# VincentGourbin/ltx-video-swift-mlx

Measured on NVIDIA B200. Metric: dit_steps_per_s, higher is better.
Workload: dtype bf16

## Files before the change

ltx-video-swift-mlx_b200/csrc/api.cu:

```cuda
#include <cstring>

#include "ctx.h"

using namespace ltx;

namespace {

thread_local std::string g_create_error;

template <typename Fn>
int guarded(ltx_ctx* c, Fn&& fn) {
  if (!c) return LTX_ERR_INVALID_ARGUMENT;
  try {
    LTX_CUDA(cudaSetDevice(c->device));
    fn();
    return LTX_OK;
  } catch (const LtxError& e) {
    c->last_error = e.what();
    return e.code;
  } catch (const std::exception& e) {
    c->last_error = e.what();
    return LTX_ERR_CUDA;
  }
}
// ... 63 lines not shown
  }
  if (it == c->graphs.end()) {
    if (c->graphs.size() >= 8) {
      auto lru = c->graphs.begin();
      for (auto j = c->graphs.begin(); j != c->graphs.end(); ++j)
        if (j->second.last_use < lru->second.last_use) lru = j;
      graph_destroy(lru->second);
      c->graphs.erase(lru);
    }
    StepGraph g;
    g.last_use = ++c->graph_clock;
    c->graphs[key] = g;
    body();
    return;
  }
  StepGraph& g = it->second;
  g.last_use = ++c->graph_clock;
  if (g.state < 0) { body(); return; }
  if (g.state == 0) {
    const uint64_t gen = devbuf_generation().load();
    const uint64_t l0 = c->launches;
    cudaGraph_t graph = nullptr;
    bool ok = cudaStreamBeginCapture(c->stream, cudaStreamCaptureModeRelaxed) == cudaSuccess;
    if (ok) {
      try {
        body();
      } catch (...) {
        cudaStreamEndCapture(c->stream, &graph);
        if (graph) cudaGraphDestroy(graph);
        cudaGetLastError();
        g.state = -1;
        throw;
      }
      ok = cudaStreamEndCapture(c->stream, &graph) == cudaSuccess && graph != nullptr;
    }
    const uint64_t n_launch = c->launches - l0;
    if (ok && devbuf_generation().load() == gen) ok = cudaGraphInstantiate(&g.exec, graph, 0) == cudaSuccess;
    else ok = false;
    if (graph) cudaGraphDestroy(graph);
    if (!ok) {
      cudaGetLastError();
      graph_destroy(g);
      g.state = -1;
      c->launches = l0;
      body();
      return;
    }
    g.state = 1;
    g.generation = gen;
    g.launches = n_launch;
    c->graph_captures++;
    LTX_CUDA(cudaGraphLaunch(g.exec, c->stream));
    return;
  }
  c->launches += g.launches;
  c->graph_replays++;
  LTX_CUDA(cudaGraphLaunch(g.exec, c->stream));
}

const TextCache* find_text(const TextCache* slots, uint64_t key, int B, int S) {
  if (key == 0) return nullptr;
  for (int i = 0; i < 2; ++i)
    if (slots[i].key == key && slots[i].B == B && slots[i].S == S) return &slots[i];
  return nullptr;
}

}

namespace ltx {
void graphs_clear(ltx_ctx* c) {
  for (auto& kv : c->graphs) graph_destroy(kv.second);
  c->graphs.clear();
}
}

extern "C" {

const char* ltx_version(void) { return "ltxcuda 0.1.0 (sm_100a)"; }

void ltx_config_default(ltx_config* cfg) {
  if (!cfg) return;
  cfg->num_layers = 48;
  cfg->num_heads = 32;
  cfg->head_dim = 128;
  cfg->in_channels = 128;
  cfg->out_channels = 128;
  cfg->caption_channels = 3840;
  cfg->ffn_mult = 4;
  cfg->rope_theta = 10000.0f;
  cfg->max_pos[0] = 20;
  cfg->max_pos[1] = 2048;
  cfg->max_pos[2] = 2048;
  cfg->timestep_scale_multiplier = 1000.0f;
  cfg->norm_eps = 1e-6f;
  cfg->vae_latent_channels = 128;
  cfg->vae_base_channels = 1024;
  cfg->vae_blocks_per_stage = 5;
  cfg->vae_patch_size = 4;
  cfg->vae_encoder_base_channels = 128;
  cfg->upscaler_mid_channels = 1024;
  cfg->upscaler_blocks = 4;
  cfg->audio_num_heads = 32;
  cfg->audio_head_dim = 64;
  cfg->audio_in_channels = 128;
  cfg->audio_max_pos = 20;
}

int ltx_ctx_create(const ltx_config* cfg, int device, ltx_ctx** out) {
  if (!cfg || !out) return LTX_ERR_INVALID_ARGUMENT;
  *out = nullptr;
  try {
    int ndev = 0;
    cudaError_t e = cudaGetDeviceCount(&ndev);
    LTX_CHECK(e == cudaSuccess && ndev > 0, LTX_ERR_CUDA, "no CUDA device available (libltxcuda has no CPU fallback)");
    LTX_CHECK(device >= 0 && device < ndev, LTX_ERR_INVALID_ARGUMENT, "bad device index");
    cudaDeviceProp prop;
    LTX_CUDA(cudaGetDeviceProperties(&prop, device));
    LTX_CHECK(prop.major == 10, LTX_ERR_CUDA,
              std::string("libltxcuda requires an sm_100a (Blackwell) device, found ") + prop.name);
    LTX_CHECK(cfg->head_dim == 128, LTX_ERR_INVALID_CONFIGURATION, "head_dim must be 128");
    LTX_CHECK(cfg->num_layers > 0 && cfg->num_heads > 0 && cfg->ffn_mult > 0, LTX_ERR_INVALID_CONFIGURATION,
              "bad transformer configuration");
    LTX_CUDA(cudaSetDevice(device));
    ltx_ctx* c = new ltx_ctx();
    c->cfg = *cfg;
    c->device = device;
    LTX_CUDA(cudaStreamCreateWithFlags(&c->stream, cudaStreamNonBlocking));
    *out = c;
    return LTX_OK;
  } catch (const LtxError& e) {
    g_create_error = e.what();
    return e.code;
  } catch (const std::exception& e) {
    g_create_error = e.what();
    return LTX_ERR_CUDA;
  }
}

int ltx_ctx_destroy(ltx_ctx* c) {
  if (!c) return LTX_OK;
  cudaSetDevice(c->device);
  cudaStreamSynchronize(c->stream);
  graphs_clear(c);
  try { dist_destroy(c); } catch (...) {}
  for (auto& kv : c->tensors)
    if (kv.second.ptr) cudaFree(kv.second.ptr);
  for (void* p : c->owned) cudaFree(p);
  DevBuf* bufs[] = {&c->sp_send, &c->sp_recv, &c->sp_vt, &c->sp_vel, &c->api_lat, &c->api_ctx, &c->lat_in, &c->ctx_in, &c->ts_in, &c->mask_in, &c->x, &c->xb, &c->h, &c->qk, &c->vt, &c->att, &c->q2,
                    &c->ffh, &c->vel, &c->se, &c->t1, &c->emb, &c->ada, &c->c1, &c->c2, &c->rope_cos, &c->rope_sin,
                    &c->scratch, &c->s_latent, &c->s_tok, &c->s_vc, &c->s_vu, &c->s_vs, &c->s_vprev, &c->s_ctx_pos,
                    &c->s_ctx_neg, &c->s_mask_pos, &c->s_mask_neg, &c->s_ctx_pair, &c->s_mask_pair, &c->s_sigma, &c->v_a, &c->v_b, &c->v_h, &c->v_pad,
                    &c->v_lat, &c->v_noise, &c->v_frames, &c->v_mix, &c->v_te, &c->v_split, &c->v_pad2, &c->snap_x, &c->s_ts, &c->f_asplit, &c->f_wsplit, &c->f_h,
                    &c->f_q, &c->f_k, &c->f_v, &c->f_att, &c->f_ffh, &c->f_ctx, &c->f_c1, &c->f_c2, &c->f_tk, &c->f_tv, &c->f_lat,
                    &c->f_bias, &c->q_panel, &c->gemm_ws, &c->u_part, &c->u_ab, &c->u_stats, &c->u_in, &c->u_out, &c->u_ref, &c->av.ws, &c->av.a_cos, &c->av.a_sin, &c->av.xv_cos, &c->av.xv_sin, &c->av_in[0], &c->av_in[1], &c->av_in[2], &c->av_in[3], &c->av_in[4], &c->av_in[5], &c->av_in[6], &c->av_in[7],
                    &c->v_tile_lat, &c->v_tile_noise, &c->v_tile_frames, &c->s_alat, &c->s_avc, &c->s_avu, &c->s_actx_pos, &c->s_actx_neg, &c->s_alat_pair, &c->s_actx_pair};
  for (DevBuf* b : bufs) b->release();
  for (auto& t : c->text) { t.k.release(); t.vt.release(); t.bias.release(); }
  for (auto& t : c->av.text) { t.k.release(); t.vt.release(); t.bias.release(); }
  cudaStreamDestroy(c->stream);
  delete c;
  return LTX_OK;
}

const char* ltx_last_error(const ltx_ctx* c) { return c ? c->last_error.c_str() : g_create_error.c_str(); }

int ltx_sync(ltx_ctx* c) {
  return guarded(c, [&] { LTX_CUDA(cudaStreamSynchronize(c->stream)); });
}

uint64_t ltx_launch_count(const ltx_ctx* c) { return c ? c->launches : 0; }

int ltx_host_alloc(void** ptr, size_t bytes) {
  if (!ptr || bytes == 0) return LTX_ERR_INVALID_ARGUMENT;
  *ptr = nullptr;
  return cudaHostAlloc(ptr, bytes, cudaHostAllocDefault) == cudaSuccess ? LTX_OK : LTX_ERR_CUDA;
}

int ltx_host_free(void* ptr) {
  if (!ptr) return LTX_OK;
  return cudaFreeHost(ptr) == cudaSuccess ? LTX_OK : LTX_ERR_CUDA;
}

int ltx_dist_get_unique_id(void* id_out_128) {
  if (!id_out_128) return LTX_ERR_INVALID_ARGUMENT;
  try {
    dist_get_unique_id(id_out_128);
    return LTX_OK;
  } catch (const LtxError& e) {
    g_create_error = e.what();
    return e.code;
  }
}

int ltx_dist_init(ltx_ctx* c, const void* unique_id_128, int rank, int world_size, int sp_size, int pass_groups) {
  return guarded(c, [&] {
    graphs_clear(c);
    LTX_CHECK(unique_id_128 != nullptr, LTX_ERR_INVALID_ARGUMENT, "null unique id");
    dist_init(c, unique_id_128, rank, world_size, sp_size, pass_groups);
  });
}

int ltx_dist_init_local(ltx_ctx** contexts, int n, int sp_size, int pass_groups) {
  if (!contexts || n < 1 || !contexts[0]) return LTX_ERR_INVALID_ARGUMENT;
  return guarded(contexts[0], [&] {
    for (int i = 0; i < n; ++i)
      if (contexts[i]) graphs_clear(contexts[i]);
    dist_init_local(contexts, n, sp_size, pass_groups);
  });
}

int ltx_dist_shutdown(ltx_ctx* c) {
  return guarded(c, [&] {
    graphs_clear(c);
    LTX_CUDA(cudaStreamSynchronize(c->stream));
    dist_destroy(c);
  });
}

int ltx_dist_info(const ltx_ctx* c, int* rank, int* world_size, int* sp_size, int* pass_groups) {
  if (!c) return LTX_ERR_INVALID_ARGUMENT;
  if (rank) *rank = c->dist.rank;
  if (world_size) *world_size = c->dist.world;
  if (sp_size) *sp_size = c->dist.sp;
  if (pass_groups) *pass_groups = c->dist.groups;
  return LTX_OK;
}

int ltx_dist_p2p_active(const ltx_ctx* c) { return (c && c->dist.p2p) ? 1 : 0; }

int ltx_get_stream(ltx_ctx* c, void** stream) {
  return guarded(c, [&] {
    LTX_CHECK(stream != nullptr, LTX_ERR_INVALID_ARGUMENT, "null out pointer");
    *stream = reinterpret_cast<void*>(c->stream);
  });
}

int ltx_set_graphs(ltx_ctx* c, int enabled) {
  return guarded(c, [&] {
    c->graphs_enabled = enabled ? 1 : 0;
    if (!enabled) graphs_clear(c);
  });
}

int ltx_graph_stats(const ltx_ctx* c, uint64_t* captures, uint64_t* replays) {
  if (!c) return LTX_ERR_INVALID_ARGUMENT;
  if (captures) *captures = c->graph_captures;
  if (replays) *replays = c->graph_replays;
  return LTX_OK;
}

int ltx_set_profiling(ltx_ctx* c, int enabled) {
  return guarded(c, [&] {
    LTX_CUDA(cudaStreamSynchronize(c->stream));
    for (auto& r : c->prof_recs) { c->prof_pool.push_back(r.a); c->prof_pool.push_back(r.b); }
    c->prof_recs.clear();
    c->prof_on = enabled != 0;
  });
}

int ltx_get_profile(ltx_ctx* c, double* ms, double* flops, double* bytes, uint64_t* counts, int n_classes) {
  return guarded(c, [&] {
    LTX_CHECK(ms && flops && bytes && counts && n_classes >= PROF_NCLASS, LTX_ERR_INVALID_ARGUMENT, "bad profile buffers");
    LTX_CUDA(cudaStreamSynchronize(c->stream));
    for (int i = 0; i < n_classes; ++i) { ms[i] = 0; flops[i] = 0; bytes[i] = 0; counts[i] = 0; }
    for (auto& r : c->prof_recs) {
      float t = 0.f;
      LTX_CUDA(cudaEventElapsedTime(&t, r.a, r.b));
      ms[r.cls] += t; flops[r.cls] += r.flops; bytes[r.cls] += r.bytes; counts[r.cls] += 1;
      c->prof_pool.push_back(r.a); c->prof_pool.push_back(r.b);
    }
    c->prof_recs.clear();
  });
}

int ltx_load_tensor(ltx_ctx* c, const char* key, const void* host_data, ltx_dtype dtype, const int64_t* shape, int ndim) {
  return guarded(c, [&] {
    LTX_CHECK(key != nullptr, LTX_ERR_INVALID_ARGUMENT, "null key");
    load_tensor_host(c, key, host_data, dtype, shape, ndim);
  });
}

int ltx_load_safetensors(ltx_ctx* c, const char* path, int which, int* n_loaded) {
  return guarded(c, [&] {
    const int n = load_safetensors(c, path, which);
    if (n_loaded) *n_loaded = n;
    static const char* kWhat[] = {"", "transformer", "VAE decoder", "VAE encoder", "upscaler", "audio/video transformer"};
    LTX_CHECK(n > 0, LTX_ERR_WEIGHTS, std::string("no ") + kWhat[which] + " tensors found in '" + (path ? path : "") + "'");
  });
}

int ltx_map_weight_key(int which, const char* file_key, char* out, size_t cap) {
  if (!file_key || !out || cap == 0 || which < 1 || which > 6) return LTX_ERR_INVALID_ARGUMENT;
  try {
    const std::string m = which == 1   ? map_transformer_key(file_key)
                          : which == 2 ? map_vae_key(file_key)
                          : which == 3 ? map_vae_encoder_key(file_key)
                          : which == 4 ? map_upscaler_key(file_key)
                          : which == 5 ? map_transformer_key(file_key, true)
                                       : map_lora_key(file_key);
    if (m.size() + 1 > cap) return LTX_ERR_INVALID_ARGUMENT;
    memcpy(out, m.c_str(), m.size() + 1);
    return LTX_OK;
  } catch (...) {
    return LTX_ERR_WEIGHTS;
  }
}

// ... 739 lines not shown
  });
}

int ltx_upscale_latent_dev(ltx_ctx* c, const float* latent, int F, int H, int W, float* out) {
  return guarded(c, [&] { upscale_latent_dev(c, latent, F, H, W, out); });
}

int ltx_upscale_latent(ltx_ctx* c, const float* latent, int F, int H, int W, float* out) {
  return guarded(c, [&] {
    LTX_CHECK(latent && out && F >= 1 && H > 1 && W > 1, LTX_ERR_INVALID_ARGUMENT, "bad upscale_latent arguments");
    const size_t n = static_cast<size_t>(c->cfg.vae_latent_channels) * F * H * W;
    h2d(c, c->u_in, latent, n * 4);
    c->u_out.reserve(4 * n * 4);
    upscale_latent_dev(c, c->u_in.as<float>(), F, H, W, c->u_out.as<float>());
    LTX_CUDA(cudaMemcpyAsync(out, c->u_out.ptr, 4 * n * 4, cudaMemcpyDeviceToHost, c->stream));
    LTX_CUDA(cudaStreamSynchronize(c->stream));
  });
}

int ltx_adain_filter_dev(ltx_ctx* c, float* latent, size_t n_per_channel, const float* reference, size_t n_ref_per_channel,
                         int channels, float factor) {
  return guarded(c, [&] {
    adain_filter_dev(c, latent, static_cast<int64_t>(n_per_channel), reference, static_cast<int64_t>(n_ref_per_channel), channels,
                     factor);
  });
}

int ltx_adain_filter(ltx_ctx* c, float* latent, size_t n_per_channel, const float* reference, size_t n_ref_per_channel, int channels,
                     float factor) {
  return guarded(c, [&] {
    LTX_CHECK(latent && reference && channels > 0, LTX_ERR_INVALID_ARGUMENT, "bad adain arguments");
    h2d(c, c->u_in, latent, n_per_channel * channels * 4);
    h2d(c, c->u_ref, reference, n_ref_per_channel * channels * 4);
    adain_filter_dev(c, c->u_in.as<float>(), static_cast<int64_t>(n_per_channel), c->u_ref.as<float>(),
                     static_cast<int64_t>(n_ref_per_channel), channels, factor);
    LTX_CUDA(cudaMemcpyAsync(latent, c->u_in.ptr, n_per_channel * channels * 4, cudaMemcpyDeviceToHost, c->stream));
    LTX_CUDA(cudaStreamSynchronize(c->stream));
  });
}

int ltx_op_gemm(ltx_ctx* c, const void* A, const void* B, const float* bias, void* C, int M, int N, int K, int mode,
                int force_bn) {
  return guarded(c, [&] {
    GemmEpi e;
    e.mode = mode; e.out = C; e.ldo = N; e.bias = bias;
    LTX_CHECK(mode == EPI_BF16 || mode == EPI_GELU_BF16 || mode == EPI_F32 || mode == EPI_SILU_BF16, LTX_ERR_INVALID_ARGUMENT, "bad mode");
    if (force_bn == -1) {
      LTX_CHECK(gemm_skinny_eligible(K, K, M, N, K, e, 0), LTX_ERR_INVALID_ARGUMENT, "shape not eligible for the skinny GEMM");
      launch_gemm_skinny(reinterpret_cast<const bf16*>(A), K, reinterpret_cast<const bf16*>(B), K, M, N, K, e, c->stream);
    } else if (force_bn == -2 || force_bn == -3) {
      LTX_CHECK(gemm_swapab_eligible(K, K, M, N, K, e), LTX_ERR_INVALID_ARGUMENT, "shape not eligible for the swap-AB GEMM");
      if (force_bn == -2) gemm_attach_workspace(c, e);
      launch_gemm_swapab(reinterpret_cast<const bf16*>(A), K, reinterpret_cast<const bf16*>(B), K, M, N, K, e, c->stream);
    } else {
      launch_gemm(reinterpret_cast<const bf16*>(A), K, reinterpret_cast<const bf16*>(B), K, M, N, K, e, c->stream, force_bn);
    }
    c->launches++;
  });
}

int ltx_op_gemm_blocked(ltx_ctx* c, const void* A, const void* B, const float* bias, void* plain_out, void* blocks_out, int M, int N,
                        int K, int col_from, int col_block, int64_t block_stride, int force_bn) {
  return guarded(c, [&] {
    LTX_CHECK(col_block > 0 && col_from >= 0 && col_from < N && (N - col_from) % col_block == 0 && (N - col_from) / col_block <= LTX_MAX_PEERS,
              LTX_ERR_INVALID_ARGUMENT, "bad column blocking");
    GemmEpi e;
    e.mode = EPI_BF16; e.out = plain_out; e.ldo = col_from > 0 ? col_from : col_block; e.bias = bias;
    e.col_block = col_block; e.col_block_from = col_from; e.blocked_ld = col_block; e.use_col_ptrs = 1;
    for (int j = 0; j < (N - col_from) / col_block; ++j)
      e.col_ptrs.p[j] = reinterpret_cast<bf16*>(blocks_out) + static_cast<int64_t>(j) * block_stride;
    if (force_bn == -2) {
      gemm_attach_workspace(c, e);
      launch_gemm_swapab(reinterpret_cast<const bf16*>(A), K, reinterpret_cast<const bf16*>(B), K, M, N, K, e, c->stream);
    } else {
      launch_gemm(reinterpret_cast<const bf16*>(A), K, reinterpret_cast<const bf16*>(B), K, M, N, K, e, c->stream, force_bn);
    }
    c->launches++;
  });
}

int ltx_op_gemm_resid(ltx_ctx* c, const void* A, const void* B, const float* bias, float* x, const float* gate_a,
                      const float* gate_b, void* shadow, int M, int N, int K, float scale) {
  return guarded(c, [&] {
    GemmEpi e;
    e.mode = EPI_GATE_RESID; e.resid = x; e.ldr = N; e.bias = bias; e.gate_a = gate_a; e.gate_b = gate_b; e.gate_ld = 0;
    e.rows_per_gate = M > 0 ? M : 1; e.shadow = reinterpret_cast<bf16*>(shadow); e.lds = N; e.scale = scale;
    if (M > 32 && M <= 512) gemm_attach_workspace(c, e);
    launch_gemm(reinterpret_cast<const bf16*>(A), K, reinterpret_cast<const bf16*>(B), K, M, N, K, e, c->stream, 0, 0, 0,
                32 );
    c->launches++;
  });
}

int ltx_op_gemm_skinny(ltx_ctx* c, const void* A, const void* B, const float* bias, void* out, float* x, const float* gate_a,
                       const float* gate_b, int rows_per_gate, int M, int N, int K, int mode, int items, int64_t vt_item_ld) {
  return guarded(c, [&] {
    LTX_CHECK(A && B && (mode == EPI_GATE_RESID ? x != nullptr : out != nullptr) && (items == 1 || items == 2) &&
                  (vt_item_ld == 0 || (M % items == 0 && vt_item_ld >= M / items)),
              LTX_ERR_INVALID_ARGUMENT, "bad skinny GEMM arguments");
    LTX_CHECK(mode >= EPI_BF16 && mode <= EPI_SILU_BF16 && (vt_item_ld == 0 || mode == EPI_BF16), LTX_ERR_INVALID_ARGUMENT, "bad mode");
    GemmEpi e;
    e.mode = mode; e.bias = bias;
    if (mode == EPI_GATE_RESID) {
      e.resid = x; e.ldr = N; e.gate_a = gate_a; e.gate_b = gate_b; e.gate_ld = N;
      e.rows_per_gate = rows_per_gate > 0 ? rows_per_gate : M;
    } else if (vt_item_ld > 0) {
      e.out = out; e.ldo = items * vt_item_ld; e.transpose_out = 1;
      if (items > 1) { e.t_item_rows = M / items; e.t_item_ld = vt_item_ld; }
    } else {
      e.out = out; e.ldo = N;
    }
    LTX_CHECK(gemm_skinny_eligible(K, K, M, N, K, e, 0, 32 * items), LTX_ERR_INVALID_ARGUMENT, "shape not eligible for the skinny GEMM");
    launch_gemm(reinterpret_cast<const bf16*>(A), K, reinterpret_cast<const bf16*>(B), K, M, N, K, e, c->stream, 0, 0, 0, 32 * items);
    c->launches++;
  });
}

int ltx_op_quantize(ltx_ctx* c, const void* w_bf16, int N, int K, int bits, void* q_out, float* scales_out, float* biases_out) {
  return guarded(c, [&] {
    launch_quantize(reinterpret_cast<const bf16*>(w_bf16), N, K, bits, reinterpret_cast<uint8_t*>(q_out), scales_out, biases_out,
                    c->stream);
    c->launches++;
  });
}

int ltx_op_dequantize(ltx_ctx* c, const void* q, const float* scales, const float* biases, int N, int K, int bits, void* w_bf16) {
  return guarded(c, [&] {
    QuantW W;
    W.q = reinterpret_cast<const uint8_t*>(q); W.scales = scales; W.biases = biases; W.bits = bits; W.n = N; W.k = K;
    launch_dequantize(W, reinterpret_cast<bf16*>(w_bf16), c->stream);
    c->launches++;
  });
}

int ltx_op_gemm_q(ltx_ctx* c, const void* A, const void* q, const float* scales, const float* biases, int bits, const float* bias,
                  void* C, int M, int N, int K, int mode, int force_bn) {
  return guarded(c, [&] {
    LTX_CHECK(mode == EPI_BF16 || mode == EPI_GELU_BF16 || mode == EPI_F32, LTX_ERR_INVALID_ARGUMENT, "bad mode");
    QuantW W;
    W.q = reinterpret_cast<const uint8_t*>(q); W.scales = scales; W.biases = biases; W.bits = bits; W.n = N; W.k = K;
    GemmEpi e;
    e.mode = mode; e.out = C; e.ldo = N; e.bias = bias;
    launch_gemm_q(reinterpret_cast<const bf16*>(A), K, W, M, N, K, e, c->stream, force_bn);
    c->launches++;
  });
}

int ltx_op_attention(ltx_ctx* c, const void* Q, const void* K, const void* Vt, int64_t ldvb, const float* key_bias, void* O,
                     int B, int H, int Nq, int Nk, float scale) {
  return guarded(c, [&] {
    const int D = H * 128;
    launch_attention(reinterpret_cast<const bf16*>(Q), D, reinterpret_cast<const bf16*>(K), D,
                     reinterpret_cast<const bf16*>(Vt), ldvb, key_bias, reinterpret_cast<bf16*>(O), D, B, H, Nq, Nk, D, scale,
                     c->stream);
    c->launches++;
  });
}

int ltx_op_attention_hd(ltx_ctx* c, const void* Q, const void* K, const void* Vt, int64_t ldvb, const float* key_bias, void* O,
                        int B, int H, int head_dim, int Nq, int Nk, float scale) {
  return guarded(c, [&] {
    LTX_CHECK(head_dim == 128 || head_dim == 64, LTX_ERR_UNSUPPORTED, "head_dim must be 128 or 64");
    const int D = H * head_dim;
    launch_attention(reinterpret_cast<const bf16*>(Q), D, reinterpret_cast<const bf16*>(K), D,
                     reinterpret_cast<const bf16*>(Vt), ldvb, key_bias, reinterpret_cast<bf16*>(O), D, B, H, Nq, Nk, D, scale,
                     c->stream);
    c->launches++;
  });
}

int ltx_op_attention_blocks(ltx_ctx* c, const void* Q, const void* K, const void* Vt, int64_t ldvb, int H, int Nq, int Nk,
                            float scale, void* const* o_blocks, int n_blocks, int rows_per_block) {
  return guarded(c, [&] {
    LTX_CHECK(o_blocks && n_blocks >= 1 && n_blocks <= LTX_MAX_PEERS && rows_per_block > 0 && n_blocks * rows_per_block >= Nq,
              LTX_ERR_INVALID_ARGUMENT, "bad output blocks");
    const int D = H * 128;
    PeerTable t = {};
    for (int i = 0; i < n_blocks; ++i) t.p[i] = o_blocks[i];
    launch_attention(reinterpret_cast<const bf16*>(Q), D, reinterpret_cast<const bf16*>(K), D, reinterpret_cast<const bf16*>(Vt), ldvb,
                     nullptr, reinterpret_cast<bf16*>(o_blocks[0]), D, 1, H, Nq, Nk, D, scale, c->stream, &t, rows_per_block);
    c->launches++;
  });
}

int ltx_op_rmsnorm_mod(ltx_ctx* c, const float* x, void* out_bf16, int M, int D, const float* tbl_shift,
                       const float* tbl_scale, const float* ada_shift, const float* ada_scale, float eps, int layernorm) {
  return guarded(c, [&] {
    launch_rmsnorm_mod(x, reinterpret_cast<bf16*>(out_bf16), M, D, tbl_shift, tbl_scale, ada_shift, ada_scale, 0, M, eps,
                       layernorm, c->stream);
    c->launches++;
  });
}

int ltx_op_qknorm_rope(ltx_ctx* c, void* x_bf16, int M, int D, const float* w, const float* cos_tab, const float* sin_tab,
                       int rows_per_rope, float eps) {
  return guarded(c, [&] {
    launch_qknorm_rope(reinterpret_cast<bf16*>(x_bf16), D, M, D, w, cos_tab, sin_tab, rows_per_rope, eps, c->stream);
    c->launches++;
  });
}

int ltx_conv3d_plan(int T, int H, int W, int Cin, int Cout, int mode, int ntaps, int sm_count, int32_t* plan7) {
  if (plan7 == nullptr || T <= 0 || H <= 1 || W <= 1 || Cin <= 0 || Cout <= 0 || (ntaps != 27 && ntaps != 9) || sm_count <= 0 || mode < 0 ||
      mode > 4)
    return LTX_ERR_INVALID_ARGUMENT;
  const ConvPlan p = conv3d_plan(T, H, W, Cin, Cout, mode, ntaps, true, sm_count, conv3d_pair_default(), conv3d_slab_default());
  plan7[0] = p.bn; plan7[1] = p.pair; plan7[2] = p.slab; plan7[3] = p.bt; plan7[4] = p.bh; plan7[5] = p.bw; plan7[6] = p.ksplit;
  return LTX_OK;
}

int ltx_op_conv3d(ltx_ctx* c, const float* x, const void* w, const float* bias, float* out, int T, int H, int W, int Cin,
                  int Cout, int causal) {
  return guarded(c, [&] {
    c->v_pad.reserve(static_cast<size_t>(T + 2) * (H + 2) * (W + 2) * Cin * 2);
    launch_vae_prep(x, c->v_pad.as<bf16>(), T, H, W, Cin, 0, nullptr, nullptr, causal, c->stream);
    ConvEpi e;
    e.mode = 0; e.out = out; e.bias = bias; e.resid = nullptr; e.Cin = Cin;
    float* scratch = nullptr;
    const size_t slab3 = static_cast<size_t>(3) * T * H * W * Cout * 4;
    if (conv3d_wants_tap_split(H, W, Cin, Cout)) {
      c->v_split.reserve(slab3);
      scratch = c->v_split.as<float>();
    }
    launch_conv3d(c->v_pad.as<bf16>(), reinterpret_cast<const bf16*>(w), T, H, W, Cin, Cout, e, c->stream, 27, scratch, scratch ? slab3 : 0);
    c->launches += 2;
  });
}

int ltx_op_vae_prep(ltx_ctx* c, const float* x, void* out_pad, int T, int H, int W, int C, int mode, const float* a, const float* b,
                    int pad) {
  return guarded(c, [&] {
    launch_vae_prep(x, reinterpret_cast<bf16*>(out_pad), T, H, W, C, mode, a, b, pad, c->stream);
    c->launches++;
  });
}

int ltx_op_vae_halo_fill(ltx_ctx* c, void* vol, int T, int H, int W, int C, int pad) {
  return guarded(c, [&] {
    launch_vae_halo_fill(reinterpret_cast<bf16*>(vol), T, H, W, C, pad, c->stream);
    c->launches++;
  });
}

int ltx_op_conv3d_epi(ltx_ctx* c, const void* x_pad, const void* w, const float* bias, int T, int H, int W, int Cin, int Cout,
                      int ntaps, int mode, float* out, const float* resid, int t_shift, int no_clip, void* next_pad,
                      const float* next_scale, const float* next_shift, int next_tshift) {
  return guarded(c, [&] {
    ConvEpi e;
    e.mode = mode; e.out = out; e.bias = bias; e.resid = resid; e.Cin = Cin; e.t_shift = t_shift; e.no_clip = no_clip;
    e.next_pad = reinterpret_cast<bf16*>(next_pad); e.next_scale = next_scale; e.next_shift = next_shift; e.next_tshift = next_tshift;
    float* scratch = nullptr;
    const size_t slab3 = static_cast<size_t>(3) * T * H * W * Cout * 4;
    if (mode == 0 && ntaps == 27 && conv3d_wants_tap_split(H, W, Cin, Cout)) {
      c->v_split.reserve(slab3);
      scratch = c->v_split.as<float>();
    }
    launch_conv3d(reinterpret_cast<const bf16*>(x_pad), reinterpret_cast<const bf16*>(w), T, H, W, Cin, Cout, e, c->stream, ntaps,
                  scratch, scratch ? slab3 : 0);
    c->launches++;
  });
}

}
```

ltx-video-swift-mlx_b200/csrc/attention.cu:

```cuda
#include <cstdio>
#include <cstdlib>
#include <type_traits>

#include "ltx_internal.h"
#include "ptx.cuh"

namespace ltx {

namespace {

constexpr int ATT_THREADS = 192;
constexpr int TQ = 128, TK = 64;
constexpr uint32_t ATT_TMEM_COLS = 256;
constexpr float RESCALE_THRESHOLD = 8.0f;

template <int HD, bool PAIR>
struct AttCfg {
  static constexpr int KROWS = PAIR ? TK / 2 : TK;
  static constexpr int VROWS = PAIR ? HD / 2 : HD;
  static constexpr uint32_t Q_TILE = 128 * HD * 2;
  static constexpr uint32_t Q_HALF = 128 * 64 * 2;
  static constexpr uint32_t K_TILE = KROWS * HD * 2;
  static constexpr uint32_t K_HALF = KROWS * 64 * 2;
  static constexpr uint32_t V_TILE = VROWS * TK * 2;
  static constexpr size_t SMEM = 1024 + Q_TILE + 2 * K_TILE + 2 * V_TILE + 16 * 8 + 16;
};

struct AttnParams {
  int B, H, Nq, Nk;
  float scale_log2;
  const float* key_bias;
  bf16* O;
  int64_t ldo;
  int o_rows_per_block;
  PeerTable o_blocks;
};

__device__ __forceinline__ float ex2_approx(float x) {
  float y;
  asm("ex2.approx.ftz.f32 %0, %1;" : "=f"(y) : "f"(x));
  return y;
}

template <int HD, bool PAIR>
__global__ void __launch_bounds__(ATT_THREADS, 2)
attention_fwd_tcgen05(const __grid_constant__ CUtensorMap tmQ, const __grid_constant__ CUtensorMap tmK,
                      const __grid_constant__ CUtensorMap tmV, const AttnParams p) {
  using Cfg = AttCfg<HD, PAIR>;
  extern __shared__ uint8_t smem_raw[];
  uint8_t* smem = reinterpret_cast<uint8_t*>((reinterpret_cast<uintptr_t>(smem_raw) + 1023) & ~static_cast<uintptr_t>(1023));
  uint8_t* sQ = smem;
  uint8_t* sK = sQ + Cfg::Q_TILE;
  uint8_t* sV = sK + 2 * Cfg::K_TILE;
  uint64_t* bars = reinterpret_cast<uint64_t*>(sV + 2 * Cfg::V_TILE);
  uint64_t* q_full = bars;
  uint64_t* k_full = bars + 1;
  uint64_t* v_full = bars + 5;
  uint64_t* v_empty = bars + 7;
  uint64_t* s_full = bars + 9;
  uint64_t* p_full = bars + 11;
  uint32_t* tmem_slot = reinterpret_cast<uint32_t*>(bars + 15);

  const int warp = threadIdx.x >> 5;
  const int lane = threadIdx.x & 31;
  const int q_tile = blockIdx.x, h = blockIdx.y, b = blockIdx.z;
  const int n_kv = (p.Nk + TK - 1) / TK;
  const uint32_t rank = PAIR ? cluster_ctarank() : 0;
  const bool leader = rank == 0;

  if (warp == 0 && lane == 0) {
    tma_prefetch_desc(&tmQ);
    tma_prefetch_desc(&tmK);
    tma_prefetch_desc(&tmV);
    mbar_init(q_full, PAIR ? 2 : 1);
    for (int i = 0; i < 2; ++i) {
      mbar_init(&k_full[i], PAIR ? 2 : 1);
      mbar_init(&v_full[i], PAIR ? 2 : 1);
      mbar_init(&v_empty[i], 1);
      mbar_init(&s_full[i], 1);
      mbar_init(&p_full[i], PAIR ? 8 : 4);
    }
    fence_mbar_init();
  }
  if (warp == 1) {
    if (PAIR) tmem_alloc_2cta<ATT_TMEM_COLS>(tmem_slot);
    else tmem_alloc<ATT_TMEM_COLS>(tmem_slot);
  }
  tc_fence_before();
  if (PAIR) cluster_sync_all();
  else __syncthreads();
  tc_fence_after();
  const uint32_t tmem_base = *tmem_slot;
  if (PAIR && !leader && threadIdx.x == 0) {
    uint32_t remote_addr, theirs;
    asm volatile("mapa.shared::cluster.u32 %0, %1, 0;" : "=r"(remote_addr) : "r"(smem_u32(tmem_slot)));
    asm volatile("ld.shared::cluster.u32 %0, [%1];" : "=r"(theirs) : "r"(remote_addr) : "memory");
    if (theirs != tmem_base) {
      printf("ltxcuda: attention pair got asymmetric tensor-memory columns (%u vs %u)\n", theirs, tmem_base);
      __trap();
    }
  }
  griddep_launch();
  griddep_wait();

  if (warp == 0) {
    if (lane == 0) {
      auto arm = [&](uint64_t* bar, uint32_t bytes) {
        if (!PAIR) mbar_arrive_expect_tx(bar, bytes);
        else if (leader) mbar_arrive_expect_tx(bar, 2 * bytes);
        else mbar_arrive_remote(bar, 0);
      };
      auto load2 = [&](void* dst, const CUtensorMap* m, uint64_t* bar, int c0, int c1) {
        if (PAIR) tma_load_2d_2sm(dst, m, bar, c0, c1);
        else tma_load_2d(dst, m, bar, c0, c1);
      };
      arm(q_full, Cfg::Q_TILE);
#pragma unroll
      for (int hh = 0; hh < HD / 64; ++hh)
        load2(sQ + hh * Cfg::Q_HALF, &tmQ, q_full, h * HD + hh * 64, b * p.Nq + q_tile * TQ);
      int nk = 0, nv = 0;
      uint32_t spins = 0;
      while (nk < n_kv || nv < n_kv) {
        bool progress = false;
        if (nk < n_kv && mbar_test(&s_full[nk & 1], ((nk >> 1) & 1) ^ 1)) {
          uint8_t* dst = sK + (nk & 1) * Cfg::K_TILE;
          arm(&k_full[nk & 1], Cfg::K_TILE);
#pragma unroll
          for (int hh = 0; hh < HD / 64; ++hh)
            load2(dst + hh * Cfg::K_HALF, &tmK, &k_full[nk & 1], h * HD + hh * 64, b * p.Nk + nk * TK + static_cast<int>(rank) * Cfg::KROWS);
          ++nk;
          progress = true;
        }
        if (nv < n_kv && mbar_test(&v_empty[nv & 1], ((nv >> 1) & 1) ^ 1)) {
          arm(&v_full[nv & 1], Cfg::V_TILE);
          if (PAIR)
            tma_load_3d_2sm(sV + (nv & 1) * Cfg::V_TILE, &tmV, &v_full[nv & 1], nv * TK, h * HD + static_cast<int>(rank) * Cfg::VROWS, b);
          else
            tma_load_3d(sV + (nv & 1) * Cfg::V_TILE, &tmV, &v_full[nv & 1], nv * TK, h * HD, b);
          ++nv;
          progress = true;
        }
        if (progress) {
          spins = 0;
        } else if (__nanosleep(128), ++spins > (1u << 23)) {
          printf("ltxcuda: attention producer stuck block(%d,%d,%d) k %d v %d\n", blockIdx.x, blockIdx.y, blockIdx.z, nk, nv);
          __trap();
        }
      }
    }
  } else if (warp == 1) {
    if (lane == 0 && leader) {
      constexpr uint32_t idesc_s = umma_idesc_bf16(PAIR ? 256 : 128, TK);
      constexpr uint32_t idesc_o = umma_idesc_bf16(PAIR ? 256 : 128, HD);
      auto commit = [&](uint64_t* bar) {
        if (PAIR) umma_commit_2cta(bar);
        else umma_commit(bar);
      };
      const uint32_t q_addr = smem_u32(sQ);
      uint64_t qd[HD / 16], kd[2][HD / 16], vd[2][TK / 16];
#pragma unroll
      for (int kk = 0; kk < HD / 16; ++kk) {
        qd[kk] = umma_desc_sw128(q_addr + (kk >> 2) * Cfg::Q_HALF + (kk & 3) * 32);
#pragma unroll
        for (int st = 0; st < 2; ++st)
          kd[st][kk] = umma_desc_sw128(smem_u32(sK + st * Cfg::K_TILE) + (kk >> 2) * Cfg::K_HALF + (kk & 3) * 32);
      }
#pragma unroll
      for (int kk = 0; kk < TK / 16; ++kk)
#pragma unroll
        for (int st = 0; st < 2; ++st) vd[st][kk] = umma_desc_sw128(smem_u32(sV + st * Cfg::V_TILE) + kk * 32);
      auto issue_S = [&](int j, auto st_tag) {
        constexpr int st = decltype(st_tag)::value;
        mbar_wait(&k_full[st], (j >> 1) & 1);
        tc_fence_after();
#pragma unroll
        for (int kk = 0; kk < HD / 16; ++kk) {
          if (PAIR) umma_bf16_2cta(tmem_base + st * TK, qd[kk], kd[st][kk], idesc_s, kk != 0);
          else umma_bf16(tmem_base + st * TK, qd[kk], kd[st][kk], idesc_s, kk != 0);
        }
        commit(&s_full[st]);
      };
      auto issue_PV = [&](int j, auto st_tag) {
        constexpr int st = decltype(st_tag)::value;
        mbar_wait(&v_full[st], (j >> 1) & 1);
        mbar_wait(&p_full[st], (j >> 1) & 1);
        tc_fence_after();
#pragma unroll
        for (int kk = 0; kk < TK / 16; ++kk) {
          if (PAIR) umma_bf16_ts_2cta(tmem_base + 2 * TK, tmem_base + st * TK + kk * 8, vd[st][kk], idesc_o, (j | kk) != 0);
          else umma_bf16_ts(tmem_base + 2 * TK, tmem_base + st * TK + kk * 8, vd[st][kk], idesc_o, (j | kk) != 0);
        }
        commit(&v_empty[st]);
      };
      using S0 = std::integral_constant<int, 0>;
      using S1 = std::integral_constant<int, 1>;
      mbar_wait(q_full, 0);
      issue_S(0, S0{});
      if (n_kv > 1) issue_S(1, S1{});
      for (int j = 0; j < n_kv; j += 2) {
        issue_PV(j, S0{});
        if (j + 2 < n_kv) issue_S(j + 2, S0{});
        if (j + 1 < n_kv) {
          issue_PV(j + 1, S1{});
          if (j + 3 < n_kv) issue_S(j + 3, S1{});
        }
      }
    }
  } else {
    const int q = warp & 3;
    const int r_in = q * 32 + lane;
    const uint32_t lane_addr = static_cast<uint32_t>(q * 32) << 16;
    const uint32_t o_addr = tmem_base + lane_addr + 2 * TK;
    const float LOG2E = 1.4426950408889634f;
    float m_ref = -1.0e30f, l_run = 0.f;
    auto step = [&](int j, auto masked_tag) {
      constexpr bool MASKED = decltype(masked_tag)::value;
      const int st = j & 1;
      const int kv0 = j * TK;
      const int valid = min(TK, p.Nk - kv0);
      const uint32_t s_addr = tmem_base + lane_addr + st * TK;
      mbar_wait(&s_full[st], (j >> 1) & 1);
      tc_fence_after();
      uint32_t sr[2][32];
      tmem_ld32(s_addr, sr[0]);
      tmem_ld32(s_addr + 32, sr[1]);
      tmem_ld_wait();
      float s[TK];
#pragma unroll
      for (int c = 0; c < 2; ++c)
#pragma unroll
        for (int i = 0; i < 32; ++i) s[c * 32 + i] = __uint_as_float(sr[c][i]);
      if (MASKED && p.key_bias != nullptr) {
        const float inv_scale = LOG2E / p.scale_log2;
        const float* kb = p.key_bias + static_cast<int64_t>(b) * p.Nk + kv0;
        if (valid == TK && (reinterpret_cast<uintptr_t>(kb) & 15) == 0) {
#pragma unroll
          for (int i = 0; i < TK; i += 4) {
            const float4 bv = __ldg(reinterpret_cast<const float4*>(kb + i));
            s[i] = fmaf(bv.x, inv_scale, s[i]);
            s[i + 1] = fmaf(bv.y, inv_scale, s[i + 1]);
            s[i + 2] = fmaf(bv.z, inv_scale, s[i + 2]);
            s[i + 3] = fmaf(bv.w, inv_scale, s[i + 3]);
          }
        } else {
#pragma unroll
          for (int i = 0; i < TK; ++i)
            if (i < valid) s[i] = fmaf(__ldg(kb + i), inv_scale, s[i]);
        }
      }
      if (MASKED && valid < TK) {
#pragma unroll
        for (int i = 0; i < TK; ++i)
          if (i >= valid) s[i] = -INFINITY;
      }
      float mx8[8];
#pragma unroll
      for (int i = 0; i < 8; ++i) mx8[i] = s[i];
#pragma unroll
      for (int i = 8; i < TK; ++i) mx8[i & 7] = fmaxf(mx8[i & 7], s[i]);
      const float mx = fmaxf(fmaxf(fmaxf(mx8[0], mx8[1]), fmaxf(mx8[2], mx8[3])), fmaxf(fmaxf(mx8[4], mx8[5]), fmaxf(mx8[6], mx8[7])));
      const float m_new = fmaxf(m_ref, mx);
      const bool need = (m_new - m_ref) * p.scale_log2 > RESCALE_THRESHOLD;
      if (__any_sync(0xffffffffu, need)) {
        const float alpha = need ? ex2_approx((m_ref - m_new) * p.scale_log2) : 1.0f;
        if (j > 0) {
          mbar_wait(&v_empty[(j - 1) & 1], ((j - 1) >> 1) & 1);
          tc_fence_after();
          uint32_t r[32];
#pragma unroll 1
          for (int c = 0; c < HD / 32; ++c) {
            tmem_ld32(o_addr + c * 32, r);
            tmem_ld_wait();
#pragma unroll
            for (int i = 0; i < 32; ++i) r[i] = __float_as_uint(__uint_as_float(r[i]) * alpha);
            tmem_st32(o_addr + c * 32, r);
          }
        }
        l_run *= alpha;
        if (need) m_ref = m_new;
      }
      const float neg = -m_ref * p.scale_log2;
      float rs0 = 0.f, rs1 = 0.f;
      uint32_t pk[32];
#pragma unroll
      for (int t = 0; t < 32; ++t) {
        const float p0 = ex2_approx(fmaf(s[2 * t], p.scale_log2, neg));
        const float p1 = ex2_approx(fmaf(s[2 * t + 1], p.scale_log2, neg));
        rs0 += p0;
        rs1 += p1;
        pk[t] = pack_bf16(p0, p1);
      }
      tmem_st32(s_addr, pk);
      l_run += rs0 + rs1;
      tmem_st_wait();
      tc_fence_before();
      __syncwarp();
      if (lane == 0) {
        if (PAIR) mbar_arrive_remote(&p_full[st], 0);
        else mbar_arrive(&p_full[st]);
      }
    };
    {
      const bool ragged = (p.Nk % TK) != 0;
      if (p.key_bias != nullptr) {
        for (int j = 0; j < n_kv; ++j) step(j, std::true_type{});
      } else {
        const int n_full = ragged ? n_kv - 1 : n_kv;
        for (int j = 0; j < n_full; ++j) step(j, std::false_type{});
        if (ragged) step(n_kv - 1, std::true_type{});
      }
    }
    mbar_wait(&v_empty[(n_kv - 1) & 1], ((n_kv - 1) >> 1) & 1);
    tc_fence_after();
    const float inv = 1.0f / l_run;
    constexpr int ROW_BYTES = HD * 2, CPR = HD / 8;
    uint8_t* otile = sQ;
#pragma unroll 1
    for (int c = 0; c < HD / 32; ++c) {
      uint32_t r[32];
      tmem_ld32(o_addr + c * 32, r);
      tmem_ld_wait();
#pragma unroll
      for (int i = 0; i < 32; i += 8) {
        uint4 pkv = make_uint4(pack_bf16(__uint_as_float(r[i]) * inv, __uint_as_float(r[i + 1]) * inv),
                               pack_bf16(__uint_as_float(r[i + 2]) * inv, __uint_as_float(r[i + 3]) * inv),
                               pack_bf16(__uint_as_float(r[i + 4]) * inv, __uint_as_float(r[i + 5]) * inv),
                               pack_bf16(__uint_as_float(r[i + 6]) * inv, __uint_as_float(r[i + 7]) * inv));
        const int chunk = c * 4 + (i >> 3);
        *reinterpret_cast<uint4*>(otile + r_in * ROW_BYTES + ((chunk ^ (r_in & 7)) << 4)) = pkv;
      }
    }
    __syncwarp();
    constexpr int RPI = 32 / CPR;
    const int sub = lane / CPR, ch = lane % CPR;
#pragma unroll 4
    for (int i = 0; i < 32 / RPI; ++i) {
      const int rr = q * 32 + RPI * i + sub;
      const int qi = q_tile * TQ + rr;
      if (qi >= p.Nq) continue;
      const uint4 v = *reinterpret_cast<const uint4*>(otile + rr * ROW_BYTES + ((ch ^ (rr & 7)) << 4));
      bf16* orow = p.O + (static_cast<int64_t>(b) * p.Nq + qi) * p.ldo + h * HD;
      if (p.o_rows_per_block > 0)
        orow = reinterpret_cast<bf16*>(p.o_blocks.p[qi / p.o_rows_per_block]) +
               static_cast<int64_t>(qi % p.o_rows_per_block) * p.ldo + h * HD;
      *reinterpret_cast<uint4*>(orow + ch * 8) = v;
    }
  }
  tc_fence_before();
  if (PAIR) cluster_sync_all();
  else __syncthreads();
  if (warp == 1) {
    __syncwarp();
    tc_fence_after();
    if (PAIR) tmem_dealloc_2cta<ATT_TMEM_COLS>(tmem_base);
    else tmem_dealloc<ATT_TMEM_COLS>(tmem_base);
  }
}

template <int HD, bool PAIR>
void attention_launch(const bf16* Q, int64_t ldq, const bf16* K, int64_t ldk, const bf16* Vt, int64_t ldvb, const AttnParams& p,
                      int D, cudaStream_t stream) {
  using Cfg = AttCfg<HD, PAIR>;
  auto kern = attention_fwd_tcgen05<HD, PAIR>;
  ensure_dyn_smem(kern, Cfg::SMEM);
  CUtensorMap tmQ = make_tmap_2d(Q, static_cast<uint64_t>(p.B) * p.Nq, D, ldq, 128);
  CUtensorMap tmK = make_tmap_2d(K, static_cast<uint64_t>(p.B) * p.Nk, D, ldk, Cfg::KROWS);
  CUtensorMap tmV = make_tmap_3d(Vt, p.Nk, D, p.B, static_cast<uint64_t>(p.B) * ldvb, ldvb, TK, Cfg::VROWS);
  int tiles = (p.Nq + TQ - 1) / TQ;
  if (PAIR) tiles = (tiles + 1) & ~1;
  dim3 grid(tiles, p.H, p.B);
  cudaLaunchConfig_t cfg = {};
  cfg.gridDim = grid;
  cfg.blockDim = dim3(ATT_THREADS);
  cfg.dynamicSmemBytes = Cfg::SMEM;
  cfg.stream = stream;
  cudaLaunchAttribute at[2];
  int na = 0;
  if (pdl_enabled(PDL_ATTN)) {
    at[na].id = cudaLaunchAttributeProgrammaticStreamSerialization;
    at[na].val.programmaticStreamSerializationAllowed = 1;
    ++na;
  }
  if (PAIR) {
    at[na].id = cudaLaunchAttributeClusterDimension;
    at[na].val.clusterDim.x = 2; at[na].val.clusterDim.y = 1; at[na].val.clusterDim.z = 1;
    ++na;
  }
  cfg.attrs = at;
  cfg.numAttrs = na;
  LTX_CUDA(cudaLaunchKernelEx(&cfg, kern, tmQ, tmK, tmV, p));
}

}

void launch_attention(const bf16* Q, int64_t ldq, const bf16* K, int64_t ldk, const bf16* Vt, int64_t ldvb,
                      const float* key_bias, bf16* O, int64_t ldo, int B, int H, int Nq, int Nk, int D, float scale,
                      cudaStream_t stream, const PeerTable* o_blocks, int rows_per_block) {
  LTX_CHECK(D == H * 128 || D == H * 64, 2, "attention: head_dim must be 128 or 64");
  LTX_CHECK(Nq > 0 && Nk > 0 && B > 0, 2, "attention: empty problem");
  LTX_CHECK(ldvb % 8 == 0 && ldvb >= Nk, 2, "attention: V^T per-batch pitch must be a multiple of 8 and >= Nk");
  AttnParams p;
  p.B = B; p.H = H; p.Nq = Nq; p.Nk = Nk;
  p.scale_log2 = scale * 1.4426950408889634f;
  p.key_bias = key_bias;
  p.O = O;
  p.ldo = ldo;
  p.o_rows_per_block = 0;
  p.o_blocks = PeerTable{};
  if (o_blocks) {
    LTX_CHECK(B == 1 && rows_per_block > 0, 2, "attention: peer-memory output needs B == 1");
    p.o_rows_per_block = rows_per_block;
    p.o_blocks = *o_blocks;
  }
  const char* pair_str = getenv("LTX_ATT_PAIR");
  const int pair_env = pair_str ? atoi(pair_str) : -1;
  const bool pair = pair_env < 0 ? Nq >= 3072 : (pair_env != 0 && Nq > TQ);
  if (D == H * 128) {
    if (pair) attention_launch<128, true>(Q, ldq, K, ldk, Vt, ldvb, p, D, stream);
    else attention_launch<128, false>(Q, ldq, K, ldk, Vt, ldvb, p, D, stream);
  } else {
    if (pair) attention_launch<64, true>(Q, ldq, K, ldk, Vt, ldvb, p, D, stream);
    else attention_launch<64, false>(Q, ldq, K, ldk, Vt, ldvb, p, D, stream);
  }
}

}
```

ltx-video-swift-mlx_b200/csrc/ctx.h:

```cpp
#pragma once
#include <atomic>
#include <map>
#include <string>
#include <unordered_map>
#include <vector>

#include "../../include/ltxcuda.h"
#include "ltx_internal.h"

namespace ltx {

struct DevTensor {
  void* ptr = nullptr;
  int dtype = LTX_F32;
  std::vector<int64_t> shape;
  int64_t numel() const {
    int64_t n = 1;
    for (auto d : shape) n *= d;
    return n;
  }
};

inline std::atomic<uint64_t>& devbuf_generation() {
  static std::atomic<uint64_t> g{1};
// ... 34 lines not shown
  const float *b_in = nullptr, *b_out = nullptr;
};

struct TextCache {
  uint64_t key = 0;
  uint64_t fingerprint = 0;
  int B = 0, S = 0;
  int64_t ldv = 0;
  DevBuf k;
  DevBuf vt;
  DevBuf bias;
  bool has_bias = false;
};

struct TextProjW {
  const bf16 *w_c1 = nullptr, *w_c2 = nullptr;
  const float *b_c1 = nullptr, *b_c2 = nullptr;
  int D = 0;
  const void* user = nullptr;
  const AttnWeights& (*layer)(const void* user, int i) = nullptr;
};

struct ConvW {
  const bf16* w = nullptr;
  const float* b = nullptr;
  int cin = 0, cout = 0;
  int taps = 27;
};
struct VaeResBlock {
  ConvW c1, c2;
  const float* sst = nullptr;
};
struct VaeTimeEmb {
  const bf16 *w1 = nullptr, *w2 = nullptr;
  const float *b1 = nullptr, *b2 = nullptr;
  int out = 0;
};
struct VaeWeights {
  bool ready = false;
  bool has_time = false;
  float ts_mult = 1000.0f;
  VaeTimeEmb stage_te[4], last_te;
  const float *mean = nullptr, *std = nullptr;
  ConvW conv_in, conv_out;
  std::vector<std::vector<VaeResBlock>> stages;
  std::vector<ConvW> ups;
  const float* last_sst = nullptr;
};

struct AdaLnW {
  const bf16 *w1 = nullptr, *w2 = nullptr, *wl = nullptr;
  const float *b1 = nullptr, *b2 = nullptr, *bl = nullptr;
  int dim = 0, n = 0;
};
struct AvBlockW {
  const float *norm1 = nullptr, *norm2 = nullptr, *norm3 = nullptr, *a2v_norm = nullptr;
  const float *anorm1 = nullptr, *anorm2 = nullptr, *anorm3 = nullptr, *v2a_norm = nullptr;
  AttnWeights aa1, aa2, a2v, v2a;
  const bf16 *w_in = nullptr, *w_out = nullptr;
  const float *b_in = nullptr, *b_out = nullptr;
  const float *asst = nullptr;
  const float *sst_ca_v = nullptr;
  const float *sst_ca_a = nullptr;
};
struct AvWeights {
  bool ready = false;
  int Da = 0, Ha = 0, hd = 0, Cin = 0;
  const bf16 *w_patch = nullptr, *w_c1 = nullptr, *w_c2 = nullptr, *w_out = nullptr;
  const float *b_patch = nullptr, *b_c1 = nullptr, *b_c2 = nullptr, *b_out = nullptr, *sst_out = nullptr;
  AdaLnW ada_a, cv_ss, cv_g, ca_ss, ca_g;
  std::vector<AvBlockW> blocks;
  TextCache text[2];
  int text_rr = 0;
  DevBuf ws;
  DevBuf a_cos, a_sin, xv_cos, xv_sin;
  int rope_ta = 0, rope_f = 0, rope_hw = 0;
};

struct EncResBlock { ConvW c1, c2; };
struct EncStage {
  std::vector<EncResBlock> res;
  ConvW down;
  int cout = 0;
};
struct EncWeights {
  bool ready = false;
  int base = 0;
  ConvW conv_in, conv_out;
  EncStage stage[4];
  std::vector<EncResBlock> mid;
};
struct GnW { const float *w = nullptr, *b = nullptr; };
struct UpsBlock { ConvW c1, c2; GnW n1, n2; };
struct UpsWeights {
  bool ready = false;
  int mid = 0, cin = 0;
  ConvW initial, up2d, final_conv;
  GnW initial_norm;
  std::vector<UpsBlock> pre, post;
};

}

namespace ltx {
struct DistState {
  bool p2p_tried = false, p2p = false;
  void* p2p_local = nullptr;
  size_t p2p_bytes = 0;
  void* p2p_peer[8] = {};
  bool p2p_ipc[8] = {};
  void* p2p_pool = nullptr;
  void* comm_world = nullptr;
  void* comm_sp = nullptr;
  bool sp_is_world = true;
  int rank = 0, world = 1, sp = 1, groups = 1, group = 0, sp_rank = 0;
};
struct StepGraph {
  int state = 0;
  cudaGraphExec_t exec = nullptr;
  uint64_t launches = 0;
  uint64_t generation = 0;
  uint64_t last_use = 0;
};
enum ProfClass { PROF_GEMM = 0, PROF_ATTN = 1, PROF_ROW = 2, PROF_CONV = 3, PROF_PREP = 4, PROF_OTHER = 5, PROF_COMM = 6, PROF_NCLASS = 8 };
struct ProfRec {
  cudaEvent_t a, b;
  int cls;
  double flops, bytes;
};
}

struct ltx_ctx {
  ltx_config cfg;
  ltx::DistState dist;
  bool prof_on = false;
  std::vector<ltx::ProfRec> prof_recs;
  std::vector<cudaEvent_t> prof_pool;

  std::map<std::string, ltx::StepGraph> graphs;
  uint64_t graph_clock = 0, graph_replays = 0, graph_captures = 0;
  int graphs_enabled = 1;

  int device = 0;
  cudaStream_t stream = nullptr;
  mutable std::string last_error;
  uint64_t launches = 0;

  std::map<std::string, ltx::DevTensor> tensors;
  std::unordered_map<const void*, ltx::QuantW> qw;
  int quant_bits = 16;
  int quant_materialise = 0;
  ltx::DevBuf q_panel;
  ltx::DevBuf gemm_ws;
  std::vector<void*> owned;
  bool dit_ready = false;
  std::vector<ltx::BlockWeights> blocks;
  const ltx::bf16 *w_patch = nullptr, *w_t1 = nullptr, *w_t2 = nullptr, *w_ada = nullptr, *w_c1 = nullptr, *w_c2 = nullptr,
                  *w_out = nullptr;
  const float *b_patch = nullptr, *b_t1 = nullptr, *b_t2 = nullptr, *b_ada = nullptr, *b_c1 = nullptr, *b_c2 = nullptr,
              *b_out = nullptr, *sst_out = nullptr;
  ltx::VaeWeights vae;
  ltx::AvWeights av;
  ltx::EncWeights enc;
  ltx::UpsWeights ups;

  ltx::DevBuf lat_in, ctx_in, ts_in, mask_in;
  ltx::DevBuf api_lat, api_ctx;
  ltx::DevBuf x, xb, h, qk, vt, att, q2, ffh, vel;
  ltx::DevBuf se, t1, emb, ada;
  ltx::DevBuf c1, c2;
  ltx::DevBuf rope_cos, rope_sin;
  int rope_f = 0, rope_h = 0, rope_w = 0;
  ltx::TextCache text[2];
  int text_rr = 0;
  ltx::DevBuf scratch;
  ltx::DevBuf sp_send, sp_recv, sp_vt, sp_vel;
  ltx::DevBuf snap_x;
  int snap_rows = 0;

  int precision = 16;
  ltx::DevBuf f_asplit, f_wsplit, f_h, f_q, f_k, f_v, f_att, f_ffh, f_ctx, f_c1, f_c2, f_tk, f_tv, f_lat, f_bias;

  ltx::DevBuf s_latent, s_tok, s_vc, s_vu, s_vs, s_vprev, s_ctx_pos, s_ctx_neg, s_mask_pos, s_mask_neg, s_sigma, s_ts;
  ltx::DevBuf s_ctx_pair, s_mask_pair;
  int s_F = 0, s_H = 0, s_W = 0, s_S = 0;
  bool s_has_neg = false, s_has_mask_pos = false, s_has_mask_neg = false;
  int s_ctx_dtype = LTX_BF16;
  uint64_t s_serial = 0;
  ltx::DevBuf s_alat, s_avc, s_avu, s_actx_pos, s_actx_neg;
  ltx::DevBuf s_alat_pair, s_actx_pair;
  int s_Ta = 0;

  ltx::DevBuf v_a, v_b, v_h, v_pad, v_lat, v_noise, v_frames, v_mix, v_te, v_split, v_pad2;
  ltx::DevBuf v_tile_lat, v_tile_noise, v_tile_frames;
  int vae_no_clip = 0;
  ltx::DevBuf av_in[8];
  ltx::DevBuf u_part, u_ab, u_stats, u_in, u_out, u_ref;
};

namespace ltx {
void gemm_attach_workspace(ltx_ctx* c, GemmEpi& e);
struct ProfScope {
  ltx_ctx* c;
  ProfRec r;
  bool on;
  ProfScope(ltx_ctx* ctx, int cls, double flops, double bytes, int launches = 1) : c(ctx), on(ctx->prof_on) {
    c->launches += launches;
    if (!on) return;
    auto get = [&]() {
      cudaEvent_t e;
      if (!c->prof_pool.empty()) { e = c->prof_pool.back(); c->prof_pool.pop_back(); }
      else LTX_CUDA(cudaEventCreate(&e));
      return e;
    };
    r.a = get(); r.b = get(); r.cls = cls; r.flops = flops; r.bytes = bytes;
    LTX_CUDA(cudaEventRecord(r.a, c->stream));
  }
  ~ProfScope() {
    if (!on) return;
    cudaEventRecord(r.b, c->stream);
    c->prof_recs.push_back(r);
  }
};
void graphs_clear(ltx_ctx* c);
void dit_finalize(ltx_ctx* c);
void dit_quantize(ltx_ctx* c, int bits);
void dit_forward_dev(ltx_ctx* c, const void* latent, int latent_dtype, const void* context, int context_dtype,
                     const float* timesteps_dev, int ts_per_token, const int32_t* mask_dev, int B, int N, int S, int F,
                     int H, int W, const ltx_dit_flags* flags, float* out_velocity_dev, int snapshot_block = -1,
                     int resume_block = -1);
void dit_clear_caches(ltx_ctx* c);
TextCache& dit_prepare_text(ltx_ctx* c, TextCache* slots, int* rr, const TextProjW& src, const void* context, int context_dtype,
                            const int32_t* mask_dev, int B, int S, uint64_t key);
void dit_build_rope(ltx_ctx* c, int F, int H, int W);
void dit_av_finalize(ltx_ctx* c);
void dit_av_forward_dev(ltx_ctx* c, const void* v_latent, int v_dtype, const void* a_latent, int a_dtype, const void* v_context,
                        const void* a_context, int ctx_dtype, const float* v_ts_dev, int v_ts_per_token, const float* a_ts_dev,
                        const int32_t* v_mask_dev, const int32_t* a_mask_dev, int B, int N, int Ta, int S, int F, int H, int W, uint64_t context_key,
                        float* out_v_dev, float* out_a_dev);
void dit_finalize_f32(ltx_ctx* c);
void dit_forward_f32(ltx_ctx* c, const void* latent, int latent_dtype, const void* context, int context_dtype,
                     const float* timesteps_dev, int ts_per_token, const int32_t* mask_dev, int B, int N, int S, int F, int H,
                     int W, const ltx_dit_flags* flags, float* out_velocity_dev);
void vae_finalize(ltx_ctx* c);
int vae_tiled_frames(int Fp, int tile_size, int overlap);
int vae_decode_tiled_dev(ltx_ctx* c, const float* latent_dev, int Fp, int Hp, int Wp, float timestep, const float* noise_dev,
                         int causal, int tile_size, int tile_overlap, float* frames_dev);
void vae_decode_dev(ltx_ctx* c, const float* latent_dev, int Fp, int Hp, int Wp, float timestep, const float* noise_dev,
                    int causal, float* frames_dev);
ConvW vae_pack_conv_keys(ltx_ctx* c, const std::string& wkey, const std::string& bkey, int64_t cout, int64_t cin,
                         int64_t cout_use, int taps);
const float* vae_vec(ltx_ctx* c, const std::string& key, int64_t n);
void vae_conv(ltx_ctx* c, const float* x, int prep_mode, const float* a, const float* b, const ConvW& w, int T, int H, int W,
              int pad, int epi_mode, float* out, const float* resid, int n_active = 1, int t_shift = 0);
void vae_encoder_finalize(ltx_ctx* c);
void vae_encode_dev(ltx_ctx* c, const float* pixels_dev, int T, int H, int W, int normalize, float* latent_dev);
void upscaler_finalize(ltx_ctx* c);
void upscale_latent_dev(ltx_ctx* c, const float* latent_dev, int F, int H, int W, float* out_dev);
void adain_filter_dev(ltx_ctx* c, float* latent_dev, int64_t n_per_channel, const float* ref_dev, int64_t n_ref_per_channel,
                      int C, float factor);
void renoise_dev(ltx_ctx* c, float* latent_dev, const float* noise_dev, int64_t n, float noise_scale);
void dist_get_unique_id(void* out128);
void dist_init(ltx_ctx* c, const void* unique_id, int rank, int world_size, int sp_size, int pass_groups);
void dist_init_local(ltx_ctx** contexts, int n, int sp_size, int pass_groups);
void dist_destroy(ltx_ctx* c);
void dist_broadcast(ltx_ctx* c, void* buf, size_t bytes, int root_world_rank);
void dist_allgather_sp(ltx_ctx* c, const void* send, void* recv, size_t bytes_per_rank);
void dist_all_to_all_sp(ltx_ctx* c, const void* const* send, void* const* recv, int n_tensors, size_t bytes_per_peer);
bool dist_p2p_ensure(ltx_ctx* c, size_t bytes);
void dist_p2p_barrier(ltx_ctx* c, int kind);
void dist_halo_exchange(ltx_ctx* c, const void* send_prev, void* recv_prev, const void* send_next, void* recv_next,
                        size_t bytes, int n_active);
std::string map_transformer_key(const std::string& file_key, bool include_audio = false);
std::string map_vae_key(const std::string& file_key);
std::string map_vae_encoder_key(const std::string& file_key);
std::string map_upscaler_key(const std::string& file_key);
int load_safetensors(ltx_ctx* c, const char* path, int which);
const DevTensor& get_tensor(ltx_ctx* c, const std::string& key);
void load_tensor_host(ltx_ctx* c, const std::string& key, const void* host, int dtype, const int64_t* shape, int ndim);
void init_random_weights(ltx_ctx* c, int which, uint64_t seed);
void fuse_lora(ltx_ctx* c, const std::string& key, const void* down_host, const void* up_host, int dtype, int rank, float scale);
std::string map_lora_key(const std::string& lora_key);
}
```

ltx-video-swift-mlx_b200/csrc/dit.cu:

```cuda
#include <algorithm>
#include <cmath>

#include "ctx.h"

namespace ltx {

namespace {

void gemm(ltx_ctx* c, const bf16* A, int64_t lda, const bf16* B, int64_t ldb, int M, int N, int K, const GemmEpi& e,
          int a_kblock = 0, int64_t a_kblock_stride = 0) {
  auto it = c->qw.empty() ? c->qw.end() : c->qw.find(B);
  const bool panel = it != c->qw.end() && it->second.scratch != nullptr && M >= 257;
  ProfScope ps(c, PROF_GEMM, 2.0 * M * N * K, 2.0 * (static_cast<double>(M) * K + static_cast<double>(N) * K + static_cast<double>(M) * N),
               panel ? 2 : 1);
  if (it != c->qw.end()) {
    launch_gemm_q(A, lda, it->second, M, N, K, e, c->stream, 0, a_kblock, a_kblock_stride);
    return;
  }
  if (M <= 512) {
    GemmEpi ew = e;
    gemm_attach_workspace(c, ew);
    launch_gemm(A, lda, B, ldb, M, N, K, ew, c->stream, 0, a_kblock, a_kblock_stride);
    return;
  }
  launch_gemm(A, lda, B, ldb, M, N, K, e, c->stream, 0, a_kblock, a_kblock_stride);
}
void v_transposed(ltx_ctx* c, const bf16* wv, const float* bv, const bf16* hrows, int rows, int D, bf16* out, int64_t ld_out,
                  bf16* tmp) {
  if (c->qw.empty() || c->qw.find(wv) == c->qw.end()) {
    GemmEpi ev;
    ev.mode = EPI_BF16; ev.out = out; ev.ldo = ld_out; ev.bias = bv; ev.bias_per_row = 1;
    gemm(c, wv, D, hrows, D, D, rows, D, ev);
    return;
  }
  GemmEpi ev;
  ev.mode = EPI_BF16; ev.out = tmp; ev.ldo = D; ev.bias = bv;
  gemm(c, hrows, D, wv, D, rows, D, D, ev);
  ProfScope ps(c, PROF_OTHER, 0.0, 4.0 * rows * D);
  launch_transpose_bf16(tmp, D, rows, D, out, ld_out, c->stream);
}
void attention(ltx_ctx* c, const bf16* Q, int64_t ldq, const bf16* K, int64_t ldk, const bf16* Vt, int64_t ldvb,
               const float* bias, bf16* O, int64_t ldo, int B, int H, int Nq, int Nk, int D, float scale,
               const PeerTable* o_blocks = nullptr, int rows_per_block = 0) {
  ProfScope ps(c, PROF_ATTN, 4.0 * B * H * static_cast<double>(Nq) * Nk * 128.0,
               2.0 * B * (2.0 * Nq + 2.0 * Nk) * D);
  launch_attention(Q, ldq, K, ldk, Vt, ldvb, bias, O, ldo, B, H, Nq, Nk, D, scale, c->stream, o_blocks, rows_per_block);
}
void norm_mod(ltx_ctx* c, const float* x, bf16* out, int M, int D, const float* ts, const float* tsc, const float* as,
              const float* asc, int64_t ada_ld, int rows_per_mod, float eps, int ln) {
  ProfScope ps(c, PROF_ROW, 0.0, static_cast<double>(M) * D * 6.0);
  launch_rmsnorm_mod(x, out, M, D, ts, tsc, as, asc, ada_ld, rows_per_mod, eps, ln, c->stream);
}
void qknorm(ltx_ctx* c, bf16* x, int64_t ld, int M, int D, const float* w, const float* cs, const float* sn, int rpr,
            float eps, const float* w_second = nullptr, const QkOut* blocked = nullptr) {
  const int segs = w_second ? 2 : 1;
  ProfScope ps(c, PROF_ROW, 0.0, segs * static_cast<double>(M) * D * (4.0 + (cs ? 4.0 : 0.0)), (D == 4096) ? 1 : segs);
  launch_qknorm_rope(x, ld, M, D, w, cs, sn, rpr, eps, c->stream, w_second, blocked);
}

const bf16* wbf(ltx_ctx* c, const std::string& k, int64_t r, int64_t cc) {
  const DevTensor& t = get_tensor(c, k);
  LTX_CHECK(t.dtype == LTX_BF16 && t.shape.size() == 2 && t.shape[0] == r && t.shape[1] == cc, LTX_ERR_WEIGHTS,
            "bad shape for '" + k + "'");
  return reinterpret_cast<const bf16*>(t.ptr);
}
const float* wf(ltx_ctx* c, const std::string& k, int64_t n) {
  const DevTensor& t = get_tensor(c, k);
  LTX_CHECK(t.dtype == LTX_F32 && t.numel() == n, LTX_ERR_WEIGHTS, "bad shape for '" + k + "'");
  return reinterpret_cast<const float*>(t.ptr);
}

void build_rope(ltx_ctx* c, int F, int H, int W) {
  if (c->rope_f == F && c->rope_h == H && c->rope_w == W && c->rope_cos.ptr) return;
  const ltx_config& g = c->cfg;
  const int D = g.num_heads * g.head_dim;
  const int half = D / 2;
  const int n_idx = std::max(1, D / 6);
  const int pad = std::max(0, half - n_idx * 3);
  const int64_t N = static_cast<int64_t>(F) * H * W;
  std::vector<float> cs(static_cast<size_t>(N) * half), sn(static_cast<size_t>(N) * half);
  std::vector<double> idx(n_idx);
  for (int i = 0; i < n_idx; ++i) {
    const double t = n_idx > 1 ? static_cast<double>(i) / (n_idx - 1) : 0.0;
    idx[i] = std::pow(static_cast<double>(g.rope_theta), t) * (M_PI / 2.0);
  }
  for (int f = 0; f < F; ++f) {
    const float ts = 8.0f, fi = static_cast<float>(f);
    const float st = std::max(fi * ts + (1.0f - ts), 0.0f), en = std::max((fi + 1.0f) * ts + (1.0f - ts), 0.0f);
    const float pt = ((st + en) / 2.0f) / 24.0f;
    for (int y = 0; y < H; ++y) {
      const float phh = static_cast<float>(y) * 32.0f + 16.0f;
      for (int x = 0; x < W; ++x) {
        const float pw = static_cast<float>(x) * 32.0f + 16.0f;
        const int64_t n = (static_cast<int64_t>(f) * H + y) * W + x;
        const double sc[3] = {static_cast<double>(pt) / g.max_pos[0] * 2.0 - 1.0,
                              static_cast<double>(phh) / g.max_pos[1] * 2.0 - 1.0,
                              static_cast<double>(pw) / g.max_pos[2] * 2.0 - 1.0};
        float* cr = &cs[static_cast<size_t>(n) * half];
        float* sr = &sn[static_cast<size_t>(n) * half];
        for (int p = 0; p < pad; ++p) { cr[p] = 1.0f; sr[p] = 0.0f; }
        for (int k = 0; k < n_idx; ++k)
          for (int d = 0; d < 3; ++d) {
            const int o = pad + k * 3 + d;
            if (o >= half) continue;
            const double a = idx[k] * sc[d];
            cr[o] = static_cast<float>(std::cos(a));
            sr[o] = static_cast<float>(std::sin(a));
          }
      }
    }
  }
  const size_t bytes = cs.size() * sizeof(float);
  c->rope_cos.reserve(bytes);
  c->rope_sin.reserve(bytes);
  LTX_CUDA(cudaMemcpyAsync(c->rope_cos.ptr, cs.data(), bytes, cudaMemcpyHostToDevice, c->stream));
  LTX_CUDA(cudaMemcpyAsync(c->rope_sin.ptr, sn.data(), bytes, cudaMemcpyHostToDevice, c->stream));
  LTX_CUDA(cudaStreamSynchronize(c->stream));
  c->rope_f = F; c->rope_h = H; c->rope_w = W;
}

int64_t round_up(int64_t v, int64_t m) { return (v + m - 1) / m * m; }

bool in_list(int v, const int32_t* lst, int n) {
  for (int i = 0; i < n; ++i)
    if (lst[i] == v) return true;
  return false;
}

}

TextCache& dit_prepare_text(ltx_ctx* c, TextCache* slots, int* rr, const TextProjW& src, const void* context, int context_dtype,
                            const int32_t* mask_dev, int B, int S, uint64_t key) {
  const ltx_config& g = c->cfg;
  const int D = src.D, L = g.num_layers, Cc = g.caption_channels;
  if (key != 0)
    for (int i = 0; i < 2; ++i)
      if (slots[i].key == key && slots[i].B == B && slots[i].S == S) return slots[i];
  int slot = -1;
  for (int i = 0; i < 2; ++i)
    if (slots[i].key == 0) { slot = i; break; }
  if (slot < 0) slot = ((*rr)++) & 1;
  TextCache& tc = slots[slot];
  const int64_t R = static_cast<int64_t>(B) * S;
  tc.key = key; tc.fingerprint = 0; tc.B = B; tc.S = S;
  tc.ldv = round_up(S, 8);
  tc.k.reserve(static_cast<size_t>(L) * R * D * 2);
  tc.vt.reserve(static_cast<size_t>(L) * D * B * tc.ldv * 2);
  cudaStream_t st = c->stream;
  const bf16* ctx_bf;
  if (context_dtype == LTX_BF16) {
    ctx_bf = reinterpret_cast<const bf16*>(context);
  } else {
    LTX_CHECK(context_dtype == LTX_F32, LTX_ERR_UNSUPPORTED, "context dtype must be bf16 or f32");
    LTX_CHECK((R * Cc) % 4 == 0, LTX_ERR_INVALID_ARGUMENT, "context size");
    c->ctx_in.reserve(static_cast<size_t>(R) * Cc * 2);
    {
      ProfScope ps(c, PROF_OTHER, 0.0, 6.0 * R * Cc);
      launch_cast_f32_bf16(reinterpret_cast<const float*>(context), c->ctx_in.as<bf16>(), R * Cc, st);
    }
    ctx_bf = c->ctx_in.as<bf16>();
  }
  c->c1.reserve(static_cast<size_t>(R) * D * 2);
  c->c2.reserve(static_cast<size_t>(R) * D * 2);
  GemmEpi e;
  e.mode = EPI_GELU_BF16; e.out = c->c1.ptr; e.ldo = D; e.bias = src.b_c1;
  gemm(c, ctx_bf, Cc, src.w_c1, Cc, static_cast<int>(R), D, Cc, e);
  e.mode = EPI_BF16; e.out = c->c2.ptr; e.bias = src.b_c2;
  gemm(c, c->c1.as<bf16>(), D, src.w_c2, D, static_cast<int>(R), D, D, e);
  for (int i = 0; i < L; ++i) {
    const AttnWeights& a = src.layer(src.user, i);
    bf16* kd = tc.k.as<bf16>() + static_cast<int64_t>(i) * R * D;
    bf16* vd = tc.vt.as<bf16>() + static_cast<int64_t>(i) * D * B * tc.ldv;
    GemmEpi ek;
    ek.mode = EPI_BF16; ek.out = kd; ek.ldo = D; ek.bias = a.bk;
    gemm(c, c->c2.as<bf16>(), D, a.wk, D, static_cast<int>(R), D, D, ek);
    qknorm(c, kd, D, static_cast<int>(R), D, a.k_norm, nullptr, nullptr, 1, g.norm_eps);
    for (int b = 0; b < B; ++b)
      v_transposed(c, a.wv, a.bv, c->c2.as<bf16>() + static_cast<int64_t>(b) * S * D, S, D, vd + b * tc.ldv, B * tc.ldv,
                   c->c1.as<bf16>());
  }
  bool any_masked = false;
  if (mask_dev) {
    std::vector<int32_t> hm(static_cast<size_t>(R));
    LTX_CUDA(cudaMemcpyAsync(hm.data(), mask_dev, static_cast<size_t>(R) * 4, cudaMemcpyDeviceToHost, st));
    LTX_CUDA(cudaStreamSynchronize(st));
    for (int32_t v : hm) any_masked |= (v == 0);
  }
  tc.has_bias = any_masked;
  if (any_masked) {
    tc.bias.reserve(static_cast<size_t>(R) * 4);
    ProfScope ps(c, PROF_OTHER, 0.0, 8.0 * R);
    launch_mask_to_bias(mask_dev, tc.bias.as<float>(), static_cast<int>(R), st);
  }
  return tc;
}

namespace {
const AttnWeights& video_text_layer(const void* user, int i) { return static_cast<const ltx_ctx*>(user)->blocks[i].a2; }
TextCache& prepare_text(ltx_ctx* c, const void* context, int context_dtype, const int32_t* mask_dev, int B, int S,
                        uint64_t key) {
  TextProjW src;
  src.w_c1 = c->w_c1; src.w_c2 = c->w_c2; src.b_c1 = c->b_c1; src.b_c2 = c->b_c2;
  src.D = c->cfg.num_heads * c->cfg.head_dim; src.user = c; src.layer = video_text_layer;
  return dit_prepare_text(c, c->text, &c->text_rr, src, context, context_dtype, mask_dev, B, S, key);
}
}

void dit_build_rope(ltx_ctx* c, int F, int H, int W) { build_rope(c, F, H, W); }

void gemm_attach_workspace(ltx_ctx* c, GemmEpi& e) {
  constexpr size_t kCounters = 16384, kPartials = static_cast<size_t>(40) << 20;
  if (!c->gemm_ws.ptr) {
    c->gemm_ws.reserve(kCounters * 4 + kPartials);
    LTX_CUDA(cudaMemsetAsync(c->gemm_ws.ptr, 0, kCounters * 4, c->stream));
  }
  e.ws_counters = c->gemm_ws.as<unsigned int>();
  e.ws_counter_count = kCounters;
  e.ws = reinterpret_cast<float*>(c->gemm_ws.as<uint8_t>() + kCounters * 4);
  e.ws_bytes = kPartials;
}

void dit_clear_caches(ltx_ctx* c) {
  c->rope_f = c->rope_h = c->rope_w = 0;
  for (auto& t : c->text) { t.key = 0; t.fingerprint = 0; t.B = t.S = 0; }
  for (auto& t : c->av.text) { t.key = 0; t.fingerprint = 0; t.B = t.S = 0; }
  c->av.rope_ta = c->av.rope_f = c->av.rope_hw = 0;
}

void dit_finalize(ltx_ctx* c) {
  const ltx_config& g = c->cfg;
  LTX_CHECK(g.head_dim == 128, LTX_ERR_INVALID_CONFIGURATION, "head_dim must be 128");
  const int64_t D = static_cast<int64_t>(g.num_heads) * g.head_dim, FF = g.ffn_mult * D;
  LTX_CHECK(g.in_channels % 8 == 0 && g.caption_channels % 8 == 0 && g.out_channels % 8 == 0, LTX_ERR_INVALID_CONFIGURATION,
            "channel counts must be multiples of 8");
  c->w_patch = wbf(c, "patchify_proj.weight", D, g.in_channels);
  c->b_patch = wf(c, "patchify_proj.bias", D);
  c->w_t1 = wbf(c, "adaln_single.emb.linear_1.weight", D, 256);
  c->b_t1 = wf(c, "adaln_single.emb.linear_1.bias", D);
  c->w_t2 = wbf(c, "adaln_single.emb.linear_2.weight", D, D);
  c->b_t2 = wf(c, "adaln_single.emb.linear_2.bias", D);
  c->w_ada = wbf(c, "adaln_single.linear.weight", 6 * D, D);
  c->b_ada = wf(c, "adaln_single.linear.bias", 6 * D);
  c->w_c1 = wbf(c, "caption_projection.linear_1.weight", D, g.caption_channels);
  c->b_c1 = wf(c, "caption_projection.linear_1.bias", D);
  c->w_c2 = wbf(c, "caption_projection.linear_2.weight", D, D);
  c->b_c2 = wf(c, "caption_projection.linear_2.bias", D);
  c->sst_out = wf(c, "scale_shift_table", 2 * D);
  c->w_out = wbf(c, "proj_out.weight", g.out_channels, D);
  c->b_out = wf(c, "proj_out.bias", g.out_channels);
  c->blocks.assign(g.num_layers, BlockWeights());
  for (int i = 0; i < g.num_layers; ++i) {
    const std::string p = "transformer_blocks." + std::to_string(i) + ".";
    BlockWeights& b = c->blocks[i];
    b.sst = wf(c, p + "scale_shift_table", 6 * D);
    {
      const bf16* wq = wbf(c, p + "attn1.to_q.weight", D, D);
      const bf16* wk = wbf(c, p + "attn1.to_k.weight", D, D);
      const bf16* wv = wbf(c, p + "attn1.to_v.weight", D, D);
      const float* bq = wf(c, p + "attn1.to_q.bias", D);
      const float* bk = wf(c, p + "attn1.to_k.bias", D);
      const float* bvv = wf(c, p + "attn1.to_v.bias", D);
      bf16* wqkv = nullptr;
      float* bqkv = nullptr;
      LTX_CUDA(cudaMalloc(&wqkv, static_cast<size_t>(3) * D * D * 2));
      c->owned.push_back(wqkv);
      LTX_CUDA(cudaMalloc(&bqkv, static_cast<size_t>(3) * D * 4));
      c->owned.push_back(bqkv);
      const bf16* ws[3] = {wq, wk, wv};
      const float* bs[3] = {bq, bk, bvv};
      for (int t = 0; t < 3; ++t) {
        LTX_CUDA(cudaMemcpyAsync(wqkv + static_cast<size_t>(t) * D * D, ws[t], static_cast<size_t>(D) * D * 2, cudaMemcpyDeviceToDevice, c->stream));
        LTX_CUDA(cudaMemcpyAsync(bqkv + static_cast<size_t>(t) * D, bs[t], static_cast<size_t>(D) * 4, cudaMemcpyDeviceToDevice, c->stream));
      }
      LTX_CUDA(cudaStreamSynchronize(c->stream));
      for (const char* k : {"attn1.to_q.weight", "attn1.to_k.weight", "attn1.to_v.weight"}) {
        auto it = c->tensors.find(p + k);
        cudaFree(it->second.ptr);
        c->tensors.erase(it);
      }
      b.a1.wq = wqkv; b.a1.wk = wqkv + D * D; b.a1.wv = wqkv + 2 * D * D;
      b.a1.bq = bqkv; b.a1.bk = bqkv + D; b.a1.bv = bqkv + 2 * D;
    }
    b.a1.wo = wbf(c, p + "attn1.to_out.weight", D, D);
    b.a1.bo = wf(c, p + "attn1.to_out.bias", D);
    b.a1.q_norm = wf(c, p + "attn1.q_norm.weight", D);
    b.a1.k_norm = wf(c, p + "attn1.k_norm.weight", D);
    b.a2.wq = wbf(c, p + "attn2.to_q.weight", D, D);
    b.a2.bq = wf(c, p + "attn2.to_q.bias", D);
    b.a2.wk = wbf(c, p + "attn2.to_k.weight", D, D);
    b.a2.bk = wf(c, p + "attn2.to_k.bias", D);
    b.a2.wv = wbf(c, p + "attn2.to_v.weight", D, D);
    b.a2.bv = wf(c, p + "attn2.to_v.bias", D);
    b.a2.wo = wbf(c, p + "attn2.to_out.weight", D, D);
    b.a2.bo = wf(c, p + "attn2.to_out.bias", D);
    b.a2.q_norm = wf(c, p + "attn2.q_norm.weight", D);
    b.a2.k_norm = wf(c, p + "attn2.k_norm.weight", D);
    b.w_in = wbf(c, p + "ff.project_in.proj.weight", FF, D);
    b.b_in = wf(c, p + "ff.project_in.proj.bias", FF);
    b.w_out = wbf(c, p + "ff.project_out.weight", D, FF);
    b.b_out = wf(c, p + "ff.project_out.bias", D);
  }
  c->scratch.reserve(64 * sizeof(double));
  c->dit_ready = true;
}

void dit_quantize(ltx_ctx* c, int bits) {
  LTX_CHECK(c->dit_ready, LTX_ERR_WEIGHTS, "DiT weights not finalized");
  LTX_CHECK(bits == 8 || bits == 4, LTX_ERR_UNSUPPORTED, "quant_bits must be 16, 8 or 4");
  const ltx_config& g = c->cfg;
  const int D = g.num_heads * g.head_dim, FF = g.ffn_mult * D;
  auto release = [&](const void* p) {
    for (auto it = c->tensors.begin(); it != c->tensors.end(); ++it)
      if (it->second.ptr == p) { cudaFree(it->second.ptr); c->tensors.erase(it); return; }
    for (auto it = c->owned.begin(); it != c->owned.end(); ++it)
      if (*it == p) { cudaFree(*it); c->owned.erase(it); return; }
  };
  std::vector<const void*> to_free;
  auto qf = [&](const bf16*& w, int N, int K) {
    LTX_CHECK(K % 64 == 0, LTX_ERR_INVALID_CONFIGURATION, "quantisation needs every Linear input width to be a multiple of 64");
    uint8_t* q = nullptr;
    float *s = nullptr, *b = nullptr;
    void* handle = nullptr;
    const size_t qbytes = static_cast<size_t>(N) * K * bits / 8, sbytes = static_cast<size_t>(K / 64) * N * 4;
    LTX_CUDA(cudaMalloc(&q, qbytes));
    LTX_CUDA(cudaMalloc(&s, sbytes));
    LTX_CUDA(cudaMalloc(&b, sbytes));
    LTX_CUDA(cudaMalloc(&handle, 16));
    c->owned.push_back(q); c->owned.push_back(s); c->owned.push_back(b); c->owned.push_back(handle);
    launch_quantize(w, N, K, bits, q, s, b, c->stream);
    QuantW r;
    r.q = q; r.scales = s; r.biases = b; r.bits = bits; r.n = N; r.k = K;
    if (c->quant_materialise) {
      launch_dequantize_panel(r, const_cast<bf16*>(w), c->stream);
      LTX_CUDA(cudaStreamSynchronize(c->stream));
      for (void* ptr : {static_cast<void*>(q), static_cast<void*>(s), static_cast<void*>(b), handle}) {
        cudaFree(ptr);
        c->owned.erase(std::find(c->owned.begin(), c->owned.end(), ptr));
      }
      return;
    }
    LTX_CUDA(cudaStreamSynchronize(c->stream));
    c->qw[handle] = r;
    to_free.push_back(w);
    w = reinterpret_cast<const bf16*>(handle);
  };
  const bool codes = !c->quant_materialise;
  qf(c->w_patch, D, g.in_channels);
  qf(c->w_c1, D, g.caption_channels);
  qf(c->w_c2, D, D);
  qf(c->w_out, g.out_channels, D);
  for (auto& b : c->blocks) {
    qf(b.a1.wq, 2 * D, D);
    if (codes) b.a1.wk = nullptr;
    qf(b.a1.wv, D, D); qf(b.a1.wo, D, D);
    qf(b.a2.wq, D, D); qf(b.a2.wk, D, D); qf(b.a2.wv, D, D); qf(b.a2.wo, D, D);
    qf(b.w_in, FF, D); qf(b.w_out, D, FF);
  }
  if (c->av.ready) {
    AvWeights& a = c->av;
    const int Da = a.Da, FFa = g.ffn_mult * Da, Ca = a.Cin;
    qf(a.w_patch, Da, Ca);
    qf(a.w_c1, Da, g.caption_channels);
    qf(a.w_c2, Da, Da);
    qf(a.w_out, Ca, Da);
    auto qattn = [&](AttnWeights& w, int qdim, int cdim, int inner) {
      qf(w.wq, inner, qdim); qf(w.wk, inner, cdim); qf(w.wv, inner, cdim); qf(w.wo, qdim, inner);
    };
    for (auto& b : a.blocks) {
      qattn(b.aa1, Da, Da, Da);
      qattn(b.aa2, Da, Da, Da);
      qattn(b.a2v, D, Da, Da);
      qattn(b.v2a, Da, D, Da);
// ... 285 lines not shown
```

ltx-video-swift-mlx_b200/csrc/dit_av.cu:

```cuda
#include <algorithm>
#include <cmath>

#include "ctx.h"
#include "ptx.cuh"

namespace ltx {

namespace {

__device__ __forceinline__ float block_sum_256(float v, float* red) {
  v = warp_sum(v);
  const int warp = threadIdx.x >> 5, lane = threadIdx.x & 31;
  __syncthreads();
  if (lane == 0) red[warp] = v;
  __syncthreads();
  float t = 0.f;
  for (int w = 0; w < (blockDim.x >> 5); ++w) t += red[w];
  return t;
}

__global__ void __launch_bounds__(256) rmsnorm_w_mod_kernel(const float* x, bf16* out, int D, const float* w, const float* sc_t,
                                                             const float* sc_a, const float* sh_t, const float* sh_a, int64_t a_ld,
                                                             int a_rpr, float eps) {
  __shared__ float red[8];
// ... 74 lines not shown
    }
  }
  auto ld4 = [](const float* p, int i, float dflt) {
    return p ? reinterpret_cast<const float4*>(p)[i] : make_float4(dflt, dflt, dflt, dflt);
  };
#pragma unroll
  for (int o = 0; o < NOUT; ++o) {
    const ModSet& m = o == 0 ? m0 : m1;
    float4 sc[VPT], sh[VPT];
    auto combine = [&](int64_t aoff) {
#pragma unroll
      for (int k = 0; k < VPT; ++k) {
        const int i = threadIdx.x + k * 256;
        const float4 ww = ld4(w, i, 1.f), a = ld4(m.sc_t, i, 0.f), b = ld4(m.sc_a ? m.sc_a + aoff : nullptr, i, 0.f),
                     cc = ld4(m.sh_t, i, 0.f), d = ld4(m.sh_a ? m.sh_a + aoff : nullptr, i, 0.f);
        sc[k] = make_float4(ww.x * (1.f + a.x + b.x), ww.y * (1.f + a.y + b.y), ww.z * (1.f + a.z + b.z), ww.w * (1.f + a.w + b.w));
        sh[k] = make_float4(cc.x + d.x, cc.y + d.y, cc.z + d.z, cc.w + d.w);
      }
    };
    if (m.a_ld == 0) combine(0);
#pragma unroll
    for (int rr = 0; rr < ROWS; ++rr) {
      const int row = row0 + rr;
      if (row >= M) break;
      if (m.a_ld != 0 && (rr == 0 || row / m.rpr != (row - 1) / m.rpr)) combine(static_cast<int64_t>(row / m.rpr) * m.a_ld);
      uint2* orow = reinterpret_cast<uint2*>(m.out + static_cast<int64_t>(row) * D);
#pragma unroll
      for (int k = 0; k < VPT; ++k)
        orow[threadIdx.x + k * 256] =
            make_uint2(pack_bf16(v[rr][k].x * s2[rr] * sc[k].x + sh[k].x, v[rr][k].y * s2[rr] * sc[k].y + sh[k].y),
                       pack_bf16(v[rr][k].z * s2[rr] * sc[k].z + sh[k].z, v[rr][k].w * s2[rr] * sc[k].w + sh[k].w));
    }
  }
}

__global__ void __launch_bounds__(256) qknorm_rope_hd_kernel(bf16* x, int64_t ld, int D, int hd, const float* w, const float* cosb,
                                                              const float* sinb, int rows_per_rope, float eps) {
  __shared__ float red[8];
  griddep_launch();
  griddep_wait();
  const int row = blockIdx.x;
  bf16* xr = x + static_cast<int64_t>(row) * ld;
  const int nchunk = D >> 3;
  float ss = 0.f;
  for (int i = threadIdx.x; i < nchunk; i += blockDim.x) {
    const uint4 u = reinterpret_cast<const uint4*>(xr)[i];
    const __nv_bfloat162* h2 = reinterpret_cast<const __nv_bfloat162*>(&u);
#pragma unroll
    for (int t = 0; t < 4; ++t) {
      const float2 f = __bfloat1622float2(h2[t]);
      ss += f.x * f.x + f.y * f.y;
    }
  }
  const float rstd = rsqrtf(block_sum_256(ss, red) / D + eps);
  const int half = hd >> 1, cph = half >> 3;
  const int npair = D >> 4;
  const float* cr = cosb ? cosb + static_cast<int64_t>(row % rows_per_rope) * (D >> 1) : nullptr;
  const float* sr = sinb ? sinb + static_cast<int64_t>(row % rows_per_rope) * (D >> 1) : nullptr;
  for (int pc = threadIdx.x; pc < npair; pc += blockDim.x) {
    const int hh = pc / cph, jc = (pc % cph) * 8;
    const int c1 = hh * hd + jc, c2 = c1 + half;
    const uint4 u1 = *reinterpret_cast<const uint4*>(xr + c1);
    const uint4 u2 = *reinterpret_cast<const uint4*>(xr + c2);
    const __nv_bfloat162* a2 = reinterpret_cast<const __nv_bfloat162*>(&u1);
    const __nv_bfloat162* b2 = reinterpret_cast<const __nv_bfloat162*>(&u2);
    float x1[8], x2[8], y1[8], y2[8];
#pragma unroll
    for (int t = 0; t < 4; ++t) {
      const float2 fa = __bfloat1622float2(a2[t]), fb = __bfloat1622float2(b2[t]);
      x1[2 * t] = fa.x * rstd * w[c1 + 2 * t];
      x1[2 * t + 1] = fa.y * rstd * w[c1 + 2 * t + 1];
      x2[2 * t] = fb.x * rstd * w[c2 + 2 * t];
      x2[2 * t + 1] = fb.y * rstd * w[c2 + 2 * t + 1];
    }
    if (cr) {
      const int fi = hh * half + jc;
#pragma unroll
      for (int t = 0; t < 8; ++t) {
        const float cs = cr[fi + t], sn = sr[fi + t];
        y1[t] = x1[t] * cs - x2[t] * sn;
        y2[t] = x2[t] * cs + x1[t] * sn;
      }
    } else {
#pragma unroll
      for (int t = 0; t < 8; ++t) { y1[t] = x1[t]; y2[t] = x2[t]; }
    }
    *reinterpret_cast<uint4*>(xr + c1) =
        make_uint4(pack_bf16(y1[0], y1[1]), pack_bf16(y1[2], y1[3]), pack_bf16(y1[4], y1[5]), pack_bf16(y1[6], y1[7]));
    *reinterpret_cast<uint4*>(xr + c2) =
        make_uint4(pack_bf16(y2[0], y2[1]), pack_bf16(y2[2], y2[3]), pack_bf16(y2[4], y2[5]), pack_bf16(y2[6], y2[7]));
  }
}

void gemm(ltx_ctx* c, const bf16* A, int64_t lda, const bf16* B, int64_t ldb, int M, int N, int K, const GemmEpi& e,
          int items = 1) {
  auto it = c->qw.empty() ? c->qw.end() : c->qw.find(B);
  const bool panel = it != c->qw.end() && it->second.scratch != nullptr && M >= 257;
  ProfScope ps(c, PROF_GEMM, 2.0 * M * N * K, 2.0 * (static_cast<double>(M) * K + static_cast<double>(N) * K + static_cast<double>(M) * N),
               panel ? 2 : 1);
  if (it != c->qw.end()) {
    launch_gemm_q(A, lda, it->second, M, N, K, e, c->stream);
    return;
  }
  launch_gemm(A, lda, B, ldb, M, N, K, e, c->stream, 0, 0, 0, 32 * items);
}
void linear(ltx_ctx* c, const bf16* A, int M, int K, const bf16* W, const float* b, int N, bf16* out, int mode = EPI_BF16,
            int items = 1) {
  GemmEpi e;
  e.mode = mode; e.out = out; e.ldo = N; e.bias = b;
  gemm(c, A, K, W, K, M, N, K, e, items);
}
void linear_resid(ltx_ctx* c, const bf16* A, int M, int K, const bf16* W, const float* b, int N, float* x, const float* gate_a,
                  const float* gate_b, int64_t gate_ld = 0, int gate_rows = 1, int items = 1) {
  GemmEpi e;
  e.mode = EPI_GATE_RESID; e.resid = x; e.ldr = N; e.bias = b; e.gate_a = gate_a; e.gate_b = gate_b; e.gate_ld = gate_ld;
  e.rows_per_gate = gate_ld > 0 ? gate_rows : (M > 0 ? M : 1);
  gemm(c, A, K, W, K, M, N, K, e, items);
}
void linear_t(ltx_ctx* c, const bf16* W, const float* b, int Nout, int K, const bf16* hrows, int rows, int items, bf16* out,
              int64_t item_ld, bf16* tmp) {
  const int64_t ld_out = items * item_ld;
  if (c->qw.empty() || c->qw.find(W) == c->qw.end()) {
    GemmEpi e;
    e.mode = EPI_BF16; e.out = out; e.ldo = ld_out; e.bias = b;
    if (items > 1) { e.t_item_rows = rows; e.t_item_ld = item_ld; }
    if (rows <= 32 && gemm_skinny_eligible(K, K, items * rows, Nout, K, e, 0, 32 * items)) {
      e.transpose_out = 1;
      gemm(c, hrows, K, W, K, items * rows, Nout, K, e, items);
      return;
    }
    e.t_item_rows = 0;
    e.bias_per_row = 1;
    if (items == 1 || rows == item_ld) {
      gemm(c, W, K, hrows, K, Nout, items * rows, K, e);
      return;
    }
    for (int i = 0; i < items; ++i) {
      e.out = out + i * item_ld;
      gemm(c, W, K, hrows + static_cast<int64_t>(i) * rows * K, K, Nout, rows, K, e);
    }
    return;
  }
  GemmEpi e;
  e.mode = EPI_BF16; e.out = tmp; e.ldo = Nout; e.bias = b;
  gemm(c, hrows, K, W, K, items * rows, Nout, K, e, items);
  ProfScope ps(c, PROF_OTHER, 0.0, 4.0 * items * rows * Nout, items);
  for (int i = 0; i < items; ++i)
    launch_transpose_bf16(tmp + static_cast<int64_t>(i) * rows * Nout, Nout, rows, Nout, out + i * item_ld, ld_out, c->stream);
}
void attention(ltx_ctx* c, const bf16* Q, const bf16* K, int64_t ldk, const bf16* Vt, int64_t ldv, const float* bias, bf16* O, int H,
               int hd, int B, int Nq, int Nk) {
  const int D = H * hd;
  ProfScope ps(c, PROF_ATTN, 4.0 * B * H * static_cast<double>(Nq) * Nk * hd, 2.0 * B * (2.0 * Nq + 2.0 * Nk) * D);
  launch_attention(Q, D, K, ldk, Vt, ldv, bias, O, D, B, H, Nq, Nk, D, 1.0f / sqrtf(static_cast<float>(hd)), c->stream);
}
void normw(ltx_ctx* c, const float* x, bf16* out, int M, int D, const float* w, const float* sc_t, const float* sc_a,
           const float* sh_t, const float* sh_a, float eps, int64_t a_ld = 0, int a_rpr = 1) {
  ProfScope ps(c, PROF_ROW, 0.0, static_cast<double>(M) * D * 6.0);
  const ModSet m{sc_t, sc_a, sh_t, sh_a, out, a_ld, a_rpr};
  if (D == 4096)
    launch_pdl(PDL_ROWS, rmsnorm_w_mod_fast_kernel<4, 4, 1>, dim3((M + 3) / 4), dim3(256), 0, c->stream, x, M, w, m, m, eps);
  else if (D == 2048)
    launch_pdl(PDL_ROWS, rmsnorm_w_mod_fast_kernel<2, 4, 1>, dim3((M + 3) / 4), dim3(256), 0, c->stream, x, M, w, m, m, eps);
  else
    launch_pdl(PDL_ROWS, rmsnorm_w_mod_kernel, dim3(M), dim3(256), 0, c->stream, x, out, D, w, sc_t, sc_a, sh_t, sh_a, a_ld, a_rpr,
               eps);
  LTX_CUDA(cudaGetLastError());
}
void normw2(ltx_ctx* c, const float* x, bf16* out0, bf16* out1, int M, int D, const float* w, const float* tbl, const float* ada,
            float eps, int64_t a_ld = 0, int a_rpr = 1) {
  const ModSet m0{tbl, ada, tbl + D, ada + D, out0, a_ld, a_rpr},
      m1{tbl + 2 * D, ada + 2 * D, tbl + 3 * D, ada + 3 * D, out1, a_ld, a_rpr};
  if (D == 4096 || D == 2048) {
    ProfScope ps(c, PROF_ROW, 0.0, static_cast<double>(M) * D * 8.0);
    if (D == 4096)
      launch_pdl(PDL_ROWS, rmsnorm_w_mod_fast_kernel<4, 4, 2>, dim3((M + 3) / 4), dim3(256), 0, c->stream, x, M, w, m0, m1, eps);
    else
      launch_pdl(PDL_ROWS, rmsnorm_w_mod_fast_kernel<2, 4, 2>, dim3((M + 3) / 4), dim3(256), 0, c->stream, x, M, w, m0, m1, eps);
    LTX_CUDA(cudaGetLastError());
    return;
  }
  normw(c, x, out0, M, D, w, m0.sc_t, m0.sc_a, m0.sh_t, m0.sh_a, eps, a_ld, a_rpr);
  normw(c, x, out1, M, D, w, m1.sc_t, m1.sc_a, m1.sh_t, m1.sh_a, eps, a_ld, a_rpr);
}
void qknorm_hd(ltx_ctx* c, bf16* x, int M, int D, int hd, const float* w, const float* cs, const float* sn, int rpr, float eps) {
  ProfScope ps(c, PROF_ROW, 0.0, static_cast<double>(M) * D * (4.0 + (cs ? 4.0 : 0.0)));
  launch_pdl(PDL_ROWS, qknorm_rope_hd_kernel, dim3(M), dim3(256), 0, c->stream, x, static_cast<int64_t>(D), D, hd, w, cs, sn,
             rpr > 0 ? rpr : 1, eps);
  LTX_CUDA(cudaGetLastError());
}

const bf16* wbf(ltx_ctx* c, const std::string& k, int64_t r, int64_t cc) {
  const DevTensor& t = get_tensor(c, k);
  LTX_CHECK(t.dtype == LTX_BF16 && t.shape.size() == 2 && t.shape[0] == r && t.shape[1] == cc, LTX_ERR_WEIGHTS,
            "bad shape for '" + k + "'");
  return reinterpret_cast<const bf16*>(t.ptr);
}
const float* wf(ltx_ctx* c, const std::string& k, int64_t n) {
  const DevTensor& t = get_tensor(c, k);
  LTX_CHECK(t.dtype == LTX_F32 && t.numel() == n, LTX_ERR_WEIGHTS, "bad shape for '" + k + "'");
  return reinterpret_cast<const float*>(t.ptr);
}
AttnWeights attn_w(ltx_ctx* c, const std::string& p, int64_t qdim, int64_t cdim, int64_t inner) {
  AttnWeights a;
  a.wq = wbf(c, p + ".to_q.weight", inner, qdim); a.bq = wf(c, p + ".to_q.bias", inner);
  a.wk = wbf(c, p + ".to_k.weight", inner, cdim); a.bk = wf(c, p + ".to_k.bias", inner);
  a.wv = wbf(c, p + ".to_v.weight", inner, cdim); a.bv = wf(c, p + ".to_v.bias", inner);
  a.wo = wbf(c, p + ".to_out.weight", qdim, inner); a.bo = wf(c, p + ".to_out.bias", qdim);
  a.q_norm = wf(c, p + ".q_norm.weight", inner);
  a.k_norm = wf(c, p + ".k_norm.weight", inner);
  return a;
}
AdaLnW adaln_w(ltx_ctx* c, const std::string& p, int64_t dim, int n) {
  AdaLnW a;
  a.w1 = wbf(c, p + ".emb.linear_1.weight", dim, 256); a.b1 = wf(c, p + ".emb.linear_1.bias", dim);
  a.w2 = wbf(c, p + ".emb.linear_2.weight", dim, dim); a.b2 = wf(c, p + ".emb.linear_2.bias", dim);
  a.wl = wbf(c, p + ".linear.weight", n * dim, dim); a.bl = wf(c, p + ".linear.bias", n * dim);
  a.dim = static_cast<int>(dim); a.n = n;
  return a;
}

void adaln_single(ltx_ctx* c, const AdaLnW& a, const float* se, float* t1, float* emb, float* lin, int B = 1) {
  ProfScope ps(c, PROF_OTHER, 2.0 * B * a.dim * (256.0 + (1.0 + a.n) * a.dim), 2.0 * a.dim * (256.0 + (1.0 + a.n) * a.dim), 3);
  launch_gemv(a.w1, a.b1, se, t1, B, a.dim, 256, 0, c->stream);
  launch_gemv(a.w2, a.b2, t1, emb, B, a.dim, a.dim, 1, c->stream);
  launch_gemv(a.wl, a.bl, emb, lin, B, a.n * a.dim, a.dim, 1, c->stream);
}

void adaln_single_rows(ltx_ctx* c, const AdaLnW& a, const bf16* se_bf, int R, bf16* t1_bf, float* emb, float* lin, int64_t ld_lin,
                       int items) {
  GemmEpi e1;
  e1.mode = EPI_SILU_BF16; e1.out = t1_bf; e1.ldo = a.dim; e1.bias = a.b1;
  gemm(c, se_bf, 256, a.w1, 256, R, a.dim, 256, e1, items);
  GemmEpi e2;
  e2.mode = EPI_F32; e2.out = emb; e2.ldo = a.dim; e2.bias = a.b2;
  gemm(c, t1_bf, a.dim, a.w2, a.dim, R, a.dim, a.dim, e2, items);
  {
    ProfScope ps(c, PROF_OTHER, 0.0, 6.0 * R * a.dim);
    launch_silu_cast(emb, t1_bf, static_cast<int64_t>(R) * a.dim, c->stream);
  }
  GemmEpi e3;
  e3.mode = EPI_F32; e3.out = lin; e3.ldo = ld_lin; e3.bias = a.bl;
  gemm(c, t1_bf, a.dim, a.wl, a.dim, R, a.n * a.dim, a.dim, e3, items);
}

void build_rope_1d(ltx_ctx* c, DevBuf& cosb, DevBuf& sinb, const std::vector<float>& pos, int dim, float theta, int max_pos) {
  const int half = dim / 2, n_idx = std::max(1, dim / 2);
  const size_t T = pos.size();
  std::vector<float> cs(T * half), sn(T * half);
  std::vector<double> idx(n_idx);
  for (int i = 0; i < n_idx; ++i)
    idx[i] = std::pow(static_cast<double>(theta), n_idx > 1 ? static_cast<double>(i) / (n_idx - 1) : 0.0) * (M_PI / 2.0);
  for (size_t t = 0; t < T; ++t) {
    const double sc = static_cast<double>(pos[t]) / max_pos * 2.0 - 1.0;
    for (int k = 0; k < half; ++k) {
      const double a = idx[k] * sc;
      cs[t * half + k] = static_cast<float>(std::cos(a));
      sn[t * half + k] = static_cast<float>(std::sin(a));
    }
  }
  cosb.reserve(cs.size() * 4);
  sinb.reserve(sn.size() * 4);
  LTX_CUDA(cudaMemcpyAsync(cosb.ptr, cs.data(), cs.size() * 4, cudaMemcpyHostToDevice, c->stream));
  LTX_CUDA(cudaMemcpyAsync(sinb.ptr, sn.data(), sn.size() * 4, cudaMemcpyHostToDevice, c->stream));
  LTX_CUDA(cudaStreamSynchronize(c->stream));
}

const AttnWeights& audio_text_layer(const void* user, int i) { return static_cast<const ltx_ctx*>(user)->av.blocks[i].aa2; }

int64_t round_up8(int64_t v) { return (v + 7) / 8 * 8; }

}

void dit_av_finalize(ltx_ctx* c) {
  const ltx_config& g = c->cfg;
  LTX_CHECK(c->dit_ready && c->precision == 16 && c->qw.empty(), LTX_ERR_WEIGHTS,
            "the dual model is finalized on the bf16 video weights (quantisation follows)");
  AvWeights& a = c->av;
  const int64_t D = static_cast<int64_t>(g.num_heads) * g.head_dim;
  const int Ha = g.audio_num_heads > 0 ? g.audio_num_heads : 32, hd = g.audio_head_dim > 0 ? g.audio_head_dim : 64;
  LTX_CHECK(hd == 64 || hd == 128, LTX_ERR_INVALID_CONFIGURATION, "audio_head_dim must be 64 or 128");
  const int64_t Da = static_cast<int64_t>(Ha) * hd, FFa = g.ffn_mult * Da;
  LTX_CHECK(Da % 128 == 0, LTX_ERR_INVALID_CONFIGURATION, "audio inner dim must be a multiple of 128");
  const int Ca = g.audio_in_channels > 0 ? g.audio_in_channels : 128;
  a.Da = static_cast<int>(Da); a.Ha = Ha; a.hd = hd; a.Cin = Ca;
  a.w_patch = wbf(c, "audio_patchify_proj.weight", Da, Ca); a.b_patch = wf(c, "audio_patchify_proj.bias", Da);
  a.w_c1 = wbf(c, "audio_caption_projection.linear_1.weight", Da, g.caption_channels);
  a.b_c1 = wf(c, "audio_caption_projection.linear_1.bias", Da);
  a.w_c2 = wbf(c, "audio_caption_projection.linear_2.weight", Da, Da);
  a.b_c2 = wf(c, "audio_caption_projection.linear_2.bias", Da);
  a.sst_out = wf(c, "audio_scale_shift_table", 2 * Da);
  a.w_out = wbf(c, "audio_proj_out.weight", Ca, Da); a.b_out = wf(c, "audio_proj_out.bias", Ca);
  a.ada_a = adaln_w(c, "audio_adaln_single", Da, 6);
  a.cv_ss = adaln_w(c, "av_ca_video_scale_shift_adaln_single", D, 4);
  a.cv_g = adaln_w(c, "av_ca_a2v_gate_adaln_single", D, 1);
  a.ca_ss = adaln_w(c, "av_ca_audio_scale_shift_adaln_single", Da, 4);
  a.ca_g = adaln_w(c, "av_ca_v2a_gate_adaln_single", Da, 1);
  a.blocks.assign(g.num_layers, AvBlockW());
  for (int i = 0; i < g.num_layers; ++i) {
    const std::string p = "transformer_blocks." + std::to_string(i) + ".";
    AvBlockW& b = a.blocks[i];
    b.norm1 = wf(c, p + "norm1.weight", D); b.norm2 = wf(c, p + "norm2.weight", D); b.norm3 = wf(c, p + "norm3.weight", D);
    b.a2v_norm = wf(c, p + "audio_to_video_norm.weight", D);
    b.anorm1 = wf(c, p + "audio_norm1.weight", Da); b.anorm2 = wf(c, p + "audio_norm2.weight", Da);
    b.anorm3 = wf(c, p + "audio_norm3.weight", Da); b.v2a_norm = wf(c, p + "video_to_audio_norm.weight", Da);
    b.aa1 = attn_w(c, p + "audio_attn1", Da, Da, Da);
    b.aa2 = attn_w(c, p + "audio_attn2", Da, Da, Da);
// ... 25 lines not shown
  const ltx_config& g = c->cfg;
  const int D = g.num_heads * g.head_dim, FFD = g.ffn_mult * D, Hv = g.num_heads, L = g.num_layers, hdv = g.head_dim;
  const int Da = av.Da, Ha = av.Ha, hda = av.hd, FFa = g.ffn_mult * Da, Cv = g.in_channels, Ca = av.Cin;
  const float eps = g.norm_eps;
  cudaStream_t st = c->stream;
  const int64_t ldv = round_up8(N), lda = round_up8(Ta);
  const int R = B * N, Ra = B * Ta;

  c->x.reserve(static_cast<size_t>(R) * D * 4);
  c->h.reserve(static_cast<size_t>(R) * D * 2);
  c->q2.reserve(static_cast<size_t>(R) * D * 2);
  c->qk.reserve(static_cast<size_t>(R) * 2 * D * 2);
  c->vt.reserve(static_cast<size_t>(D) * B * ldv * 2);
  c->att.reserve(static_cast<size_t>(R) * D * 2);
  c->ffh.reserve(static_cast<size_t>(R) * FFD * 2);
  c->xb.reserve(static_cast<size_t>(R) * D * 2);
  DevBuf& wsb = av.ws;
  const int VR = v_ts_per_token ? R : B;
  const bool per_item = B > 1;
  const int v_rpr = v_ts_per_token ? 1 : N;
  const int64_t vada_ld = (v_ts_per_token || per_item) ? 6 * static_cast<int64_t>(D) : 0;
  const int64_t cv_ld = v_ts_per_token ? 5 * static_cast<int64_t>(D) : per_item ? 4 * static_cast<int64_t>(D) : 0;
  const int64_t cvg_ld = v_ts_per_token ? 5 * static_cast<int64_t>(D) : per_item ? static_cast<int64_t>(D) : 0;
  const int64_t aada_ld = per_item ? 6 * static_cast<int64_t>(Da) : 0, ca_ld = per_item ? 4 * static_cast<int64_t>(Da) : 0,
                cag_ld = per_item ? static_cast<int64_t>(Da) : 0;
  size_t off = 0;
  auto carve = [&](size_t bytes) { const size_t o = off; off += (bytes + 255) / 256 * 256; return o; };
  const size_t o_ax = carve(static_cast<size_t>(Ra) * Da * 4), o_ah = carve(static_cast<size_t>(Ra) * Da * 2),
               o_ah2 = carve(static_cast<size_t>(Ra) * Da * 2), o_aq = carve(static_cast<size_t>(Ra) * Da * 2),
               o_ak = carve(static_cast<size_t>(Ra) * Da * 2), o_avt = carve(static_cast<size_t>(Da) * B * lda * 2),
               o_aatt = carve(static_cast<size_t>(Ra) * Da * 2), o_affh = carve(static_cast<size_t>(Ra) * FFa * 2),
               o_cq = carve(static_cast<size_t>(R) * Da * 2), o_catt = carve(static_cast<size_t>(R) * Da * 2),
               o_vt2 = carve(static_cast<size_t>(Da) * B * ldv * 2),
               o_lat = carve(static_cast<size_t>(std::max(R * Cv, Ra * Ca)) * 2),
               o_se = carve(static_cast<size_t>(B) * 2 * 256 * 4), o_t1 = carve(static_cast<size_t>(B) * D * 4),
               o_vemb = carve(static_cast<size_t>(VR) * D * 4), o_aemb = carve(static_cast<size_t>(B) * Da * 4),
               o_vada = carve(static_cast<size_t>(VR) * 6 * D * 4), o_aada = carve(static_cast<size_t>(B) * 6 * Da * 4),
               o_cv = carve(static_cast<size_t>(VR) * 5 * D * 4), o_ca = carve(static_cast<size_t>(B) * 5 * Da * 4),
               o_scr = carve(static_cast<size_t>(VR) * D * 4),
               o_tq = carve(c->qw.empty() ? 0 : static_cast<size_t>(std::max(R, Ra)) * D * 2),
               o_sev = carve(v_ts_per_token ? static_cast<size_t>(R) * 256 * 2 : 0),
               o_t1v = carve(v_ts_per_token ? static_cast<size_t>(R) * D * 2 : 0);
  wsb.reserve(off);
  uint8_t* wbase = wsb.as<uint8_t>();
  float* x = c->x.as<float>();
  bf16 *h = c->h.as<bf16>(), *h2 = c->q2.as<bf16>(), *qk = c->qk.as<bf16>(), *vt = c->vt.as<bf16>(), *att = c->att.as<bf16>(),
       *ffh = c->ffh.as<bf16>(), *q2 = c->xb.as<bf16>();
  float* ax = reinterpret_cast<float*>(wbase + o_ax);
  bf16 *ah = reinterpret_cast<bf16*>(wbase + o_ah), *ah2 = reinterpret_cast<bf16*>(wbase + o_ah2),
       *aq = reinterpret_cast<bf16*>(wbase + o_aq), *ak = reinterpret_cast<bf16*>(wbase + o_ak),
       *avt = reinterpret_cast<bf16*>(wbase + o_avt), *aatt = reinterpret_cast<bf16*>(wbase + o_aatt),
       *affh = reinterpret_cast<bf16*>(wbase + o_affh), *cq = reinterpret_cast<bf16*>(wbase + o_cq),
       *catt = reinterpret_cast<bf16*>(wbase + o_catt), *vt2 = reinterpret_cast<bf16*>(wbase + o_vt2),
       *lat_bf = reinterpret_cast<bf16*>(wbase + o_lat), *tq = reinterpret_cast<bf16*>(wbase + o_tq);
  float *se = reinterpret_cast<float*>(wbase + o_se), *t1 = reinterpret_cast<float*>(wbase + o_t1),
        *vemb = reinterpret_cast<float*>(wbase + o_vemb), *aemb = reinterpret_cast<float*>(wbase + o_aemb),
        *vada = reinterpret_cast<float*>(wbase + o_vada), *aada = reinterpret_cast<float*>(wbase + o_aada),
        *cv = reinterpret_cast<float*>(wbase + o_cv), *ca = reinterpret_cast<float*>(wbase + o_ca),
        *scr = reinterpret_cast<float*>(wbase + o_scr);

  dit_build_rope(c, F, H, W);
  if (av.rope_ta != Ta || av.rope_f != F || av.rope_hw != H * W || !av.a_cos.ptr) {
    std::vector<float> pa(Ta), pv(static_cast<size_t>(N));
    for (int i = 0; i < Ta; ++i) {
      const float fi = static_cast<float>(i), sc = 4.0f, of = 1.0f;
      const float s0 = std::max(0.0f, fi * sc + of - sc), e0 = std::max(0.0f, (fi + 1.0f) * sc + of - sc);
      pa[i] = (s0 + e0) / 2.0f * 160.0f / 16000.0f;
    }
    for (int f = 0; f < F; ++f) {
      const float ts = 8.0f, fi = static_cast<float>(f);
      const float s0 = std::max(fi * ts + (1.0f - ts), 0.0f), e0 = std::max((fi + 1.0f) * ts + (1.0f - ts), 0.0f);
      const float pt = ((s0 + e0) / 2.0f) / 24.0f;
      for (int k = 0; k < H * W; ++k) pv[static_cast<size_t>(f) * H * W + k] = pt;
    }
    const int amax = g.audio_max_pos > 0 ? g.audio_max_pos : 20;
    build_rope_1d(c, av.a_cos, av.a_sin, pa, Da, g.rope_theta, amax);
    build_rope_1d(c, av.xv_cos, av.xv_sin, pv, Da, g.rope_theta, amax);
    av.rope_ta = Ta; av.rope_f = F; av.rope_hw = H * W;
  }
  const float *cos_v = c->rope_cos.as<float>(), *sin_v = c->rope_sin.as<float>();
  const float *cos_a = av.a_cos.as<float>(), *sin_a = av.a_sin.as<float>();
  const float *cos_xv = av.xv_cos.as<float>(), *sin_xv = av.xv_sin.as<float>();
  TextProjW vsrc;
  vsrc.w_c1 = c->w_c1; vsrc.w_c2 = c->w_c2; vsrc.b_c1 = c->b_c1; vsrc.b_c2 = c->b_c2; vsrc.D = D; vsrc.user = c;
  vsrc.layer = [](const void* u, int i) -> const AttnWeights& { return static_cast<const ltx_ctx*>(u)->blocks[i].a2; };
  TextCache& tcv = dit_prepare_text(c, c->text, &c->text_rr, vsrc, v_context, ctx_dtype, v_mask_dev, B, S, context_key);
  TextProjW asrc;
  asrc.w_c1 = av.w_c1; asrc.w_c2 = av.w_c2; asrc.b_c1 = av.b_c1; asrc.b_c2 = av.b_c2; asrc.D = Da; asrc.user = c;
  asrc.layer = audio_text_layer;
  TextCache& tca = dit_prepare_text(c, av.text, &av.text_rr, asrc, a_context, ctx_dtype, a_mask_dev, B, S, context_key);
  const float* vbias = tcv.has_bias ? tcv.bias.as<float>() : nullptr;
  const float* abias = tca.has_bias ? tca.bias.as<float>() : nullptr;

  auto embed = [&](const void* lat, int dt, int rows, int Cin, const bf16* w, const float* b, int Dout, float* xout, bf16* tmp) {
    const bf16* src = reinterpret_cast<const bf16*>(lat);
    if (dt == LTX_F32) {
      LTX_CHECK((static_cast<int64_t>(rows) * Cin) % 4 == 0, LTX_ERR_INVALID_ARGUMENT, "latent size");
      ProfScope ps(c, PROF_OTHER, 0.0, 6.0 * rows * Cin);
      launch_cast_f32_bf16(reinterpret_cast<const float*>(lat), lat_bf, static_cast<int64_t>(rows) * Cin, st);
      src = lat_bf;
    }
    linear(c, src, rows, Cin, w, b, Dout, tmp, EPI_BF16, B);
    ProfScope ps(c, PROF_OTHER, 0.0, 6.0 * rows * Dout);
    launch_cast_bf16_f32(tmp, xout, static_cast<int64_t>(rows) * Dout, st);
  };
  embed(v_latent, v_dtype, R, Cv, c->w_patch, c->b_patch, D, x, h);
  embed(a_latent, a_dtype, Ra, Ca, av.w_patch, av.b_patch, Da, ax, ah);

  float* se_a = se + B * 256;
  {
    ProfScope ps(c, PROF_OTHER, 0.0, 2048.0 * B, 2);
    launch_sincos_embed(v_ts_dev, g.timestep_scale_multiplier, se, B, 256, st);
    launch_sincos_embed(a_ts_dev, g.timestep_scale_multiplier, se_a, B, 256, st);
  }
  AdaLnW vmain;
  vmain.w1 = c->w_t1; vmain.b1 = c->b_t1; vmain.w2 = c->w_t2; vmain.b2 = c->b_t2; vmain.wl = c->w_ada; vmain.bl = c->b_ada;
  vmain.dim = D; vmain.n = 6;
  float* cvg = v_ts_per_token ? cv + 4 * D : cv + static_cast<int64_t>(B) * 4 * D;
  float* cag = ca + static_cast<int64_t>(B) * 4 * Da;
  if (!v_ts_per_token) {
    adaln_single(c, vmain, se, t1, vemb, vada, B);
    adaln_single(c, av.cv_ss, se, t1, scr, cv, B);
    adaln_single(c, av.cv_g, se, t1, scr, cvg, B);
  } else {
    bf16 *sev = reinterpret_cast<bf16*>(wbase + o_sev), *t1v = reinterpret_cast<bf16*>(wbase + o_t1v);
    {
      ProfScope ps(c, PROF_OTHER, 0.0, 4.0 * R + 512.0 * R);
      launch_sincos_embed(v_ts_dev, g.timestep_scale_multiplier, nullptr, R, 256, st, sev);
    }
    adaln_single_rows(c, vmain, sev, R, t1v, vemb, vada, vada_ld, B);
    adaln_single_rows(c, av.cv_ss, sev, R, t1v, scr, cv, cv_ld, B);
    adaln_single_rows(c, av.cv_g, sev, R, t1v, scr, cvg, cvg_ld, B);
  }
  adaln_single(c, av.ada_a, se_a, t1, aemb, aada, B);
  adaln_single(c, av.ca_ss, se_a, t1, scr, ca, B);
  adaln_single(c, av.ca_g, se_a, t1, scr, cag, B);

  for (int i = 0; i < L; ++i) {
    const BlockWeights& bv = c->blocks[i];
    const AvBlockW& ba = av.blocks[i];
    normw(c, x, h, R, D, ba.norm1, bv.sst + D, vada + D, bv.sst, vada, eps, vada_ld, v_rpr);
    {
      GemmEpi e;
      e.mode = EPI_BF16; e.out = qk; e.ldo = 2 * D; e.bias = bv.a1.bq;
      gemm(c, h, D, bv.a1.wq, D, R, 2 * D, D, e, B);
    }
    linear_t(c, bv.a1.wv, bv.a1.bv, D, D, h, N, B, vt, ldv, tq);
    {
      ProfScope ps(c, PROF_ROW, 0.0, 2.0 * R * D * 8.0, (D == 4096) ? 1 : 2);
      launch_qknorm_rope(qk, 2 * D, R, D, bv.a1.q_norm, cos_v, sin_v, N, eps, st, bv.a1.k_norm);
    }
    {
      ProfScope ps(c, PROF_ATTN, 4.0 * B * Hv * static_cast<double>(N) * N * hdv, 2.0 * 4.0 * R * D);
      launch_attention(qk, 2 * D, qk + D, 2 * D, vt, ldv, nullptr, att, D, B, Hv, N, N, D, 1.0f / sqrtf(static_cast<float>(hdv)), st);
    }
    linear_resid(c, att, R, D, bv.a1.wo, bv.a1.bo, D, x, vada + 2 * D, bv.sst + 2 * D, vada_ld, v_rpr, B);
    normw(c, ax, ah, Ra, Da, ba.anorm1, ba.asst + Da, aada + Da, ba.asst, aada, eps, aada_ld, Ta);
    linear(c, ah, Ra, Da, ba.aa1.wq, ba.aa1.bq, Da, aq, EPI_BF16, B);
    linear(c, ah, Ra, Da, ba.aa1.wk, ba.aa1.bk, Da, ak, EPI_BF16, B);
    linear_t(c, ba.aa1.wv, ba.aa1.bv, Da, Da, ah, Ta, B, avt, lda, tq);
    qknorm_hd(c, aq, Ra, Da, hda, ba.aa1.q_norm, cos_a, sin_a, Ta, eps);
    qknorm_hd(c, ak, Ra, Da, hda, ba.aa1.k_norm, cos_a, sin_a, Ta, eps);
    attention(c, aq, ak, Da, avt, lda, nullptr, aatt, Ha, hda, B, Ta, Ta);
    linear_resid(c, aatt, Ra, Da, ba.aa1.wo, ba.aa1.bo, Da, ax, aada + 2 * Da, ba.asst + 2 * Da, aada_ld, Ta, B);
    normw(c, x, h, R, D, ba.norm2, nullptr, nullptr, nullptr, nullptr, eps);
    linear(c, h, R, D, bv.a2.wq, bv.a2.bq, D, q2, EPI_BF16, B);
    qknorm_hd(c, q2, R, D, hdv, bv.a2.q_norm, nullptr, nullptr, 1, eps);
    attention(c, q2, tcv.k.as<bf16>() + static_cast<int64_t>(i) * B * S * D, D,
              tcv.vt.as<bf16>() + static_cast<int64_t>(i) * D * B * tcv.ldv, tcv.ldv, vbias, att, Hv, hdv, B, N, S);
    linear_resid(c, att, R, D, bv.a2.wo, bv.a2.bo, D, x, nullptr, nullptr, 0, 1, B);
    normw(c, ax, ah, Ra, Da, ba.anorm2, nullptr, nullptr, nullptr, nullptr, eps);
    linear(c, ah, Ra, Da, ba.aa2.wq, ba.aa2.bq, Da, aq, EPI_BF16, B);
    qknorm_hd(c, aq, Ra, Da, hda, ba.aa2.q_norm, nullptr, nullptr, 1, eps);
    attention(c, aq, tca.k.as<bf16>() + static_cast<int64_t>(i) * B * S * Da, Da,
              tca.vt.as<bf16>() + static_cast<int64_t>(i) * Da * B * tca.ldv, tca.ldv, abias, aatt, Ha, hda, B, Ta, S);
    linear_resid(c, aatt, Ra, Da, ba.aa2.wo, ba.aa2.bo, Da, ax, nullptr, nullptr, 0, 1, B);
    normw2(c, x, h, h2, R, D, ba.a2v_norm, ba.sst_ca_v, cv, eps, cv_ld, v_rpr);
    normw2(c, ax, ah, ah2, Ra, Da, ba.v2a_norm, ba.sst_ca_a, ca, eps, ca_ld, Ta);
    linear(c, h, R, D, ba.a2v.wq, ba.a2v.bq, Da, cq, EPI_BF16, B);
    linear(c, ah, Ra, Da, ba.a2v.wk, ba.a2v.bk, Da, ak, EPI_BF16, B);
    linear_t(c, ba.a2v.wv, ba.a2v.bv, Da, Da, ah, Ta, B, avt, lda, tq);
    qknorm_hd(c, cq, R, Da, hda, ba.a2v.q_norm, cos_xv, sin_xv, N, eps);
    qknorm_hd(c, ak, Ra, Da, hda, ba.a2v.k_norm, cos_a, sin_a, Ta, eps);
    attention(c, cq, ak, Da, avt, lda, nullptr, catt, Ha, hda, B, N, Ta);
    linear(c, ah2, Ra, Da, ba.v2a.wq, ba.v2a.bq, Da, aq, EPI_BF16, B);
    linear(c, h2, R, D, ba.v2a.wk, ba.v2a.bk, Da, cq, EPI_BF16, B);
    linear_t(c, ba.v2a.wv, ba.v2a.bv, Da, D, h2, N, B, vt2, ldv, tq);
    qknorm_hd(c, aq, Ra, Da, hda, ba.v2a.q_norm, cos_a, sin_a, Ta, eps);
    qknorm_hd(c, cq, R, Da, hda, ba.v2a.k_norm, cos_xv, sin_xv, N, eps);
    attention(c, aq, cq, Da, vt2, ldv, nullptr, aatt, Ha, hda, B, Ta, N);
    linear_resid(c, catt, R, Da, ba.a2v.wo, ba.a2v.bo, D, x, cvg, ba.sst_ca_v + 4 * D, cvg_ld, v_rpr, B);
    linear_resid(c, aatt, Ra, Da, ba.v2a.wo, ba.v2a.bo, Da, ax, cag, ba.sst_ca_a + 4 * Da, cag_ld, Ta, B);
    normw(c, x, h, R, D, ba.norm3, bv.sst + 4 * D, vada + 4 * D, bv.sst + 3 * D, vada + 3 * D, eps, vada_ld, v_rpr);
    linear(c, h, R, D, bv.w_in, bv.b_in, FFD, ffh, EPI_GELU_BF16, B);
    linear_resid(c, ffh, R, FFD, bv.w_out, bv.b_out, D, x, vada + 5 * D, bv.sst + 5 * D, vada_ld, v_rpr, B);
    normw(c, ax, ah, Ra, Da, ba.anorm3, ba.asst + 4 * Da, aada + 4 * Da, ba.asst + 3 * Da, aada + 3 * Da, eps, aada_ld, Ta);
    linear(c, ah, Ra, Da, ba.w_in, ba.b_in, FFa, affh, EPI_GELU_BF16, B);
    linear_resid(c, affh, Ra, FFa, ba.w_out, ba.b_out, Da, ax, aada + 5 * Da, ba.asst + 5 * Da, aada_ld, Ta, B);
  }
  auto head = [&](const float* xs, int rows, int Dx, const float* sst, const float* emb, int rpr, bf16* tmp, const bf16* w,
                  const float* b, int Cout, float* out) {
    {
      ProfScope ps(c, PROF_ROW, 0.0, static_cast<double>(rows) * Dx * 6.0);
      launch_rmsnorm_mod(xs, tmp, rows, Dx, sst, sst + Dx, emb, emb, Dx, rpr, eps, 1, st);
    }
    GemmEpi e;
    e.mode = EPI_F32; e.out = out; e.ldo = Cout; e.bias = b;
    gemm(c, tmp, Dx, w, Dx, rows, Cout, Dx, e, B);
  };
  head(x, R, D, c->sst_out, vemb, v_rpr, h, c->w_out, c->b_out, g.out_channels, out_v_dev);
  head(ax, Ra, Da, av.sst_out, aemb, Ta, ah, av.w_out, av.b_out, Ca, out_a_dev);
}

}
```

ltx-video-swift-mlx_b200/csrc/ltx_internal.h:

```cpp
#pragma once
#include <cuda.h>
#include <cuda_bf16.h>
#include <cuda_runtime.h>
#include <stdint.h>

#include <stdexcept>
#include <string>

namespace ltx {

typedef __nv_bfloat16 bf16;

struct LtxError : public std::runtime_error {
  int code;
  LtxError(int c, const std::string& m) : std::runtime_error(m), code(c) {}
};

#define LTX_CHECK(cond, code, msg)                                                                  \
  do {                                                                                              \
    if (!(cond)) throw ::ltx::LtxError((code), std::string(msg) + " [" #cond "] at " __FILE__ ":" + \
                                                   std::to_string(__LINE__));                       \
  } while (0)
#define LTX_CUDA(expr)                                                                                       \
  do {                                                                                                       \
    cudaError_t _e = (expr);                                                                                 \
    if (_e != cudaSuccess)                                                                                   \
      throw ::ltx::LtxError(3, std::string("CUDA error: ") + cudaGetErrorString(_e) + " in " #expr " at " + \
                                   __FILE__ ":" + std::to_string(__LINE__));                                 \
  } while (0)

bool pdl_enabled(int cls = 0);
enum { PDL_GEMM = 0, PDL_ROWS = 1, PDL_ATTN = 2, PDL_VAE = 3 };
template <typename... KArgs, typename... Args>
inline void launch_pdl(int cls, void (*kern)(KArgs...), dim3 grid, dim3 block, size_t smem, cudaStream_t stream, Args&&... args) {
  cudaLaunchConfig_t cfg = {};
  cfg.gridDim = grid;
  cfg.blockDim = block;
  cfg.dynamicSmemBytes = smem;
  cfg.stream = stream;
  cudaLaunchAttribute at[1];
  at[0].id = cudaLaunchAttributeProgrammaticStreamSerialization;
  at[0].val.programmaticStreamSerializationAllowed = 1;
  cfg.attrs = at;
  cfg.numAttrs = pdl_enabled(cls) ? 1 : 0;
  LTX_CUDA(cudaLaunchKernelEx(&cfg, kern, static_cast<KArgs>(args)...));
}

CUtensorMap make_tmap_2d(const void* base, uint64_t rows, uint64_t cols, uint64_t ld, uint32_t box_rows,
                         uint32_t box_cols = 64);
CUtensorMap make_tmap_thwc(const void* base, uint64_t T, uint64_t H, uint64_t W, uint64_t C, uint32_t bt, uint32_t bh,
                           uint32_t bw);
CUtensorMap make_tmap_3d(const void* base, uint64_t d0, uint64_t d1, uint64_t d2, uint64_t stride1, uint64_t stride2,
                         uint32_t box0, uint32_t box1);
int device_sm_count();
void ensure_dyn_smem(const void* kernel, size_t bytes);
template <typename K>
inline void ensure_dyn_smem(K* kernel, size_t bytes) { ensure_dyn_smem(reinterpret_cast<const void*>(kernel), bytes); }

enum EpiMode : int {
  EPI_BF16 = 0,
  EPI_GELU_BF16 = 1,
  EPI_GATE_RESID = 2,
  EPI_F32 = 3,
  EPI_SILU_BF16 = 4,
};

constexpr int LTX_MAX_PEERS = 8;
struct PeerTable {
  void* p[LTX_MAX_PEERS];
};

struct GemmEpi {
  int mode = EPI_BF16;
  void* out = nullptr;
  int64_t ldo = 0;
  const float* bias = nullptr;
  int bias_per_row = 0;
  float* resid = nullptr;
  int64_t ldr = 0;
  const float* gate_a = nullptr;
  const float* gate_b = nullptr;
  int64_t gate_ld = 0;
  int rows_per_gate = 1;
  bf16* shadow = nullptr;
  int64_t lds = 0;
  float scale = 1.0f;
  int col_block = 0;
  int64_t col_block_stride = 0;
  int use_col_ptrs = 0;
  PeerTable col_ptrs = {};
  int col_block_from = 0;
  void* blocked_out = nullptr;
  int64_t blocked_ld = 0;
  int tsplit_col = 0;
  bf16* out_t = nullptr;
  int64_t ldt = 0;
  int transpose_out = 0;
  int t_item_rows = 0;
  int64_t t_item_ld = 0;
  int debug = 0;
  float* ws = nullptr;
  size_t ws_bytes = 0;
  unsigned int* ws_counters = nullptr;
  size_t ws_counter_count = 0;
};

void launch_gemm(const bf16* A, int64_t lda, const bf16* B, int64_t ldb, int M, int N, int K, const GemmEpi& epi,
                 cudaStream_t stream, int force_bn = 0, int a_kblock = 0, int64_t a_kblock_stride = 0, int allow_skinny = 0);
bool gemm_skinny_eligible(int64_t lda, int64_t ldb, int M, int N, int K, const GemmEpi& epi, int a_kblock, int max_rows = 32);
void launch_gemm_skinny(const bf16* A, int64_t lda, const bf16* W, int64_t ldb, int M, int N, int K, const GemmEpi& epi,
                        cudaStream_t stream);
int gemm_fit_tile_width(int M, int N);
bool gemm_swapab_eligible(int64_t lda, int64_t ldb, int M, int N, int K, const GemmEpi& epi);
void launch_gemm_swapab(const bf16* A, int64_t lda, const bf16* W, int64_t ldb, int M, int N, int K, const GemmEpi& epi,
                        cudaStream_t stream, int a_kblock = 0, int64_t a_kblock_stride = 0);
void launch_gemm_2cta(const bf16* A, int64_t lda, const bf16* B, int64_t ldb, int M, int N, int K, const GemmEpi& epi,
                      cudaStream_t stream, int force_bn, int a_kblock, int64_t a_kblock_stride);
int gemm2_fit_tile_width(int M, int N);
struct QuantW {
  const uint8_t* q = nullptr;
  const float* scales = nullptr;
  const float* biases = nullptr;
  int bits = 0, n = 0, k = 0;
  bf16* scratch = nullptr;
};
void launch_gemm_q(const bf16* A, int64_t lda, const QuantW& W, int M, int N, int K, const GemmEpi& epi, cudaStream_t stream,
                   int force_bn = 0, int a_kblock = 0, int64_t a_kblock_stride = 0);
void launch_quantize(const bf16* w, int N, int K, int bits, uint8_t* q, float* scales, float* biases, cudaStream_t s);
void launch_dequantize(const QuantW& W, bf16* w, cudaStream_t s);
void launch_dequantize_panel(const QuantW& W, bf16* w, cudaStream_t s);
CUtensorMap make_tmap_u8(const void* base, uint64_t rows, uint64_t row_bytes, uint32_t box_rows, uint32_t box_bytes);
void launch_transpose_bf16(const bf16* in, int64_t ld_in, int R, int C, bf16* out, int64_t ld_out, cudaStream_t s);

void launch_attention(const bf16* Q, int64_t ldq, const bf16* K, int64_t ldk, const bf16* Vt, int64_t ldvb,
                      const float* key_bias, bf16* O, int64_t ldo, int B, int H, int Nq, int Nk, int D, float scale,
                      cudaStream_t stream, const PeerTable* o_blocks = nullptr, int rows_per_block = 0);

void launch_rmsnorm_mod(const float* x, bf16* out, int M, int D, const float* tbl_shift, const float* tbl_scale,
                        const float* ada_shift, const float* ada_scale, int64_t ada_ld, int rows_per_mod, float eps,
                        int layernorm, cudaStream_t s);
struct QkOut {
  bf16* out[2] = {nullptr, nullptr};
  int heads_per_block = 0;
  int64_t block_stride = 0, ld = 0;
  int use_peer = 0;
  PeerTable peer[2] = {};
};
void launch_qknorm_rope(bf16* x, int64_t ld, int M, int D, const float* w, const float* cosb, const float* sinb,
                        int rows_per_rope, float eps, cudaStream_t s, const float* w_second = nullptr,
                        const QkOut* blocked = nullptr);
void launch_cast_f32_bf16(const float* in, bf16* out, int64_t n, cudaStream_t s);
void launch_cast_bf16_f32(const bf16* in, float* out, int64_t n, cudaStream_t s);
void launch_gemv(const bf16* W, const float* bias, const float* x, float* y, int M, int O, int I, int silu_in,
                 cudaStream_t s);
void launch_mask_to_bias(const int32_t* mask, float* bias, int n, cudaStream_t s);
void launch_scale_f32(float* x, float a, int64_t n, cudaStream_t s);
void launch_audio_cfg_euler(float* lat, const float* v_cond, const float* v_uncond, float cfg_scale, float dt, int64_t n,
                            cudaStream_t s);
void launch_sincos_embed(const float* sigma, float mult, float* out, int M, int dim, cudaStream_t s, bf16* out_bf16 = nullptr);
void launch_silu_cast(const float* in, bf16* out, int64_t n, cudaStream_t s);
void launch_fill_token_timesteps(float* ts, int n, int period, int frozen, const float* sigma_dev, cudaStream_t s);
void launch_patchify(const float* latent, bf16* tok_bf16, float* tok_f32, int C, int T, cudaStream_t s);
void launch_unpatchify(const float* tok, float* latent, int C, int T, cudaStream_t s);
void launch_transpose_slice(const float* in, int64_t ld_in, int rows, int cols, float* out, cudaStream_t s);
struct GuidedEulerArgs {
  float* latent;
  const float* v_cond;
  const float* v_uncond;
  const float* v_stg;
  float* v_prev;
  int use_prev;
  float* v_out;
  size_t n;
  float cfg, phi, stg, ge_gamma, sigma, sigma_next;
  double* scratch;
  size_t period = 0, frozen = 0;
};
void launch_guided_euler(const GuidedEulerArgs& a, cudaStream_t s);
void launch_fill_normal_bf16(bf16* p, int64_t n, float std, float mean, uint64_t seed, cudaStream_t s);
void launch_fill_normal_f32(float* p, int64_t n, float std, float mean, uint64_t seed, cudaStream_t s);

struct ConvEpi {
  int mode;
  float* out;
  const float* bias;
  const float* resid;
  int Cin;
  int t_shift = 0;
  bf16* next_pad = nullptr;
  const float* next_scale = nullptr;
  const float* next_shift = nullptr;
  int next_tshift = 1;
  int no_clip = 0;
};
bool conv3d_wants_tap_split(int H, int W, int Cin, int Cout);
struct ConvPlan {
  int bn;
  int pair;
  int slab;
  int bt, bh, bw;
  int ksplit;
};
ConvPlan conv3d_plan(int T, int H, int W, int Cin, int Cout, int mode, int ntaps, bool scratch_ok, int sm_count, bool pair_on,
                     bool slab_on);
bool conv3d_pair_default();
bool conv3d_slab_default();
void launch_conv3d(const bf16* x_pad, const bf16* w, int T, int H, int W, int Cin, int Cout, const ConvEpi& epi,
                   cudaStream_t s, int ntaps = 27, float* splitk_scratch = nullptr, size_t splitk_scratch_bytes = 0);
enum { VAE_PAD_CAUSAL = 1, VAE_PAD_ZERO_HW = 2, VAE_PAD_ZERO_T = 4 };
void launch_vae_halo_fill(bf16* pad_vol, int T, int H, int W, int C, int pad, cudaStream_t s);
void launch_vae_prep(const float* x, bf16* out, int T, int H, int W, int C, int mode, const float* a, const float* b,
                     int pad, cudaStream_t s);

}
```

Baseline: 25.66.

## Add split-KV persistent scheduling to non-paired tcgen05 attention kernel

The non-paired attention kernel becomes persistent. It walks a flat list of (batch, head, q-tile, kv-segment) work units with a grid capped at twice the SM count, and splits the KV range into up to four segments. Partial outputs and softmax stats go to a context-owned workspace and are merged using per-tile ticket counters. The aim is better SM occupancy and less launch tail when Nq is small, as in cross-attention to text or short sequences, where there are too few q-tiles per head. The cost is partial-buffer traffic, an extra merge step, and more complex barrier phase tracking across units.

```diff
diff --git a/ltx-video-swift-mlx_b200/csrc/api.cu b/ltx-video-swift-mlx_b200/csrc/api.cu
--- a/ltx-video-swift-mlx_b200/csrc/api.cu
+++ b/ltx-video-swift-mlx_b200/csrc/api.cu
@@ -239,7 +239,7 @@
                     &c->s_ctx_neg, &c->s_mask_pos, &c->s_mask_neg, &c->s_ctx_pair, &c->s_mask_pair, &c->s_sigma, &c->v_a, &c->v_b, &c->v_h, &c->v_pad,
                     &c->v_lat, &c->v_noise, &c->v_frames, &c->v_mix, &c->v_te, &c->v_split, &c->v_pad2, &c->snap_x, &c->s_ts, &c->f_asplit, &c->f_wsplit, &c->f_h,
                     &c->f_q, &c->f_k, &c->f_v, &c->f_att, &c->f_ffh, &c->f_ctx, &c->f_c1, &c->f_c2, &c->f_tk, &c->f_tv, &c->f_lat,
-                    &c->f_bias, &c->q_panel, &c->gemm_ws, &c->u_part, &c->u_ab, &c->u_stats, &c->u_in, &c->u_out, &c->u_ref, &c->av.ws, &c->av.a_cos, &c->av.a_sin, &c->av.xv_cos, &c->av.xv_sin, &c->av_in[0], &c->av_in[1], &c->av_in[2], &c->av_in[3], &c->av_in[4], &c->av_in[5], &c->av_in[6], &c->av_in[7],
+                    &c->f_bias, &c->q_panel, &c->gemm_ws, &c->attn_tickets, &c->attn_part, &c->u_part, &c->u_ab, &c->u_stats, &c->u_in, &c->u_out, &c->u_ref, &c->av.ws, &c->av.a_cos, &c->av.a_sin, &c->av.xv_cos, &c->av.xv_sin, &c->av_in[0], &c->av_in[1], &c->av_in[2], &c->av_in[3], &c->av_in[4], &c->av_in[5], &c->av_in[6], &c->av_in[7],
                     &c->v_tile_lat, &c->v_tile_noise, &c->v_tile_frames, &c->s_alat, &c->s_avc, &c->s_avu, &c->s_actx_pos, &c->s_actx_neg, &c->s_alat_pair, &c->s_actx_pair};
   for (DevBuf* b : bufs) b->release();
   for (auto& t : c->text) { t.k.release(); t.vt.release(); t.bias.release(); }
@@ -1285,7 +1285,7 @@
     const int D = H * 128;
     launch_attention(reinterpret_cast<const bf16*>(Q), D, reinterpret_cast<const bf16*>(K), D,
                      reinterpret_cast<const bf16*>(Vt), ldvb, key_bias, reinterpret_cast<bf16*>(O), D, B, H, Nq, Nk, D, scale,
-                     c->stream);
+                     attention_workspace(c, B, H, Nq, Nk, D / H), c->stream);
     c->launches++;
   });
 }
@@ -1297,7 +1297,7 @@
     const int D = H * head_dim;
     launch_attention(reinterpret_cast<const bf16*>(Q), D, reinterpret_cast<const bf16*>(K), D,
                      reinterpret_cast<const bf16*>(Vt), ldvb, key_bias, reinterpret_cast<bf16*>(O), D, B, H, Nq, Nk, D, scale,
-                     c->stream);
+                     attention_workspace(c, B, H, Nq, Nk, D / H), c->stream);
     c->launches++;
   });
 }
@@ -1311,7 +1311,8 @@
     PeerTable t = {};
     for (int i = 0; i < n_blocks; ++i) t.p[i] = o_blocks[i];
     launch_attention(reinterpret_cast<const bf16*>(Q), D, reinterpret_cast<const bf16*>(K), D, reinterpret_cast<const bf16*>(Vt), ldvb,
-                     nullptr, reinterpret_cast<bf16*>(o_blocks[0]), D, 1, H, Nq, Nk, D, scale, c->stream, &t, rows_per_block);
+                     nullptr, reinterpret_cast<bf16*>(o_blocks[0]), D, 1, H, Nq, Nk, D, scale, attention_workspace(c, 1, H, Nq, Nk, 128),
+                     c->stream, &t, rows_per_block);
     c->launches++;
   });
 }
diff --git a/ltx-video-swift-mlx_b200/csrc/attention.cu b/ltx-video-swift-mlx_b200/csrc/attention.cu
--- a/ltx-video-swift-mlx_b200/csrc/attention.cu
+++ b/ltx-video-swift-mlx_b200/csrc/attention.cu
@@ -1,3 +1,4 @@
+#include <algorithm>
 #include <cstdio>
 #include <cstdlib>
 #include <type_traits>
@@ -26,6 +27,11 @@
   static constexpr size_t SMEM = 1024 + Q_TILE + 2 * K_TILE + 2 * V_TILE + 16 * 8 + 16;
 };
 
+constexpr int MAX_SPLITS = 4;
+
+template <int HD>
+__host__ __device__ constexpr size_t part_floats() { return static_cast<size_t>(HD) * TQ + 2 * TQ; }
+
 struct AttnParams {
   int B, H, Nq, Nk;
   float scale_log2;
@@ -34,6 +40,11 @@
   int64_t ldo;
   int o_rows_per_block;
   PeerTable o_blocks;
+  int tiles;
+  int splits;
+  int units;
+  unsigned int* tickets;
+  float* partials;
 };
 
 __device__ __forceinline__ float ex2_approx(float x) {
@@ -59,14 +70,35 @@
   uint64_t* v_empty = bars + 7;
   uint64_t* s_full = bars + 9;
   uint64_t* p_full = bars + 11;
+  uint64_t* q_empty = bars + 13;
   uint32_t* tmem_slot = reinterpret_cast<uint32_t*>(bars + 15);
+  uint32_t* ticket = tmem_slot + 1;
 
   const int warp = threadIdx.x >> 5;
   const int lane = threadIdx.x & 31;
-  const int q_tile = blockIdx.x, h = blockIdx.y, b = blockIdx.z;
   const int n_kv = (p.Nk + TK - 1) / TK;
   const uint32_t rank = PAIR ? cluster_ctarank() : 0;
   const bool leader = rank == 0;
+  struct Unit { int b, h, q_tile, seg, kb, ke; };
+  auto unit_at = [&](int u) {
+    Unit w;
+    if (PAIR) {
+      w.q_tile = blockIdx.x; w.h = blockIdx.y; w.b = blockIdx.z; w.seg = 0;
+    } else {
+      w.seg = u % p.splits;
+      int t = u / p.splits;
+      w.q_tile = t % p.tiles;
+      t /= p.tiles;
+      w.h = t % p.H;
+      w.b = t / p.H;
+    }
+    w.kb = w.seg * n_kv / p.splits;
+    w.ke = (w.seg + 1) * n_kv / p.splits;
+    return w;
+  };
+  const int u_first = PAIR ? 0 : static_cast<int>(blockIdx.x);
+  const int u_end = PAIR ? 1 : p.units;
+  const int u_step = PAIR ? 1 : static_cast<int>(gridDim.x);
 
   if (warp == 0 && lane == 0) {
     tma_prefetch_desc(&tmQ);
@@ -80,6 +112,7 @@
       mbar_init(&s_full[i], 1);
       mbar_init(&p_full[i], PAIR ? 8 : 4);
     }
+    mbar_init(q_empty, 4);
     fence_mbar_init();
   }
   if (warp == 1) {
@@ -114,38 +147,52 @@
         if (PAIR) tma_load_2d_2sm(dst, m, bar, c0, c1);
         else tma_load_2d(dst, m, bar, c0, c1);
       };
-      arm(q_full, Cfg::Q_TILE);
-#pragma unroll
-      for (int hh = 0; hh < HD / 64; ++hh)
-        load2(sQ + hh * Cfg::Q_HALF, &tmQ, q_full, h * HD + hh * 64, b * p.Nq + q_tile * TQ);
-      int nk = 0, nv = 0;
-      uint32_t spins = 0;
-      while (nk < n_kv || nv < n_kv) {
-        bool progress = false;
-        if (nk < n_kv && mbar_test(&s_full[nk & 1], ((nk >> 1) & 1) ^ 1)) {
-          uint8_t* dst = sK + (nk & 1) * Cfg::K_TILE;
-          arm(&k_full[nk & 1], Cfg::K_TILE);
-#pragma unroll
-          for (int hh = 0; hh < HD / 64; ++hh)
-            load2(dst + hh * Cfg::K_HALF, &tmK, &k_full[nk & 1], h * HD + hh * 64, b * p.Nk + nk * TK + static_cast<int>(rank) * Cfg::KROWS);
-          ++nk;
-          progress = true;
-        }
-        if (nv < n_kv && mbar_test(&v_empty[nv & 1], ((nv >> 1) & 1) ^ 1)) {
-          arm(&v_full[nv & 1], Cfg::V_TILE);
-          if (PAIR)
-            tma_load_3d_2sm(sV + (nv & 1) * Cfg::V_TILE, &tmV, &v_full[nv & 1], nv * TK, h * HD + static_cast<int>(rank) * Cfg::VROWS, b);
-          else
-            tma_load_3d(sV + (nv & 1) * Cfg::V_TILE, &tmV, &v_full[nv & 1], nv * TK, h * HD, b);
-          ++nv;
-          progress = true;
-        }
-        if (progress) {
-          spins = 0;
-        } else if (__nanosleep(128), ++spins > (1u << 23)) {
-          printf("ltxcuda: attention producer stuck block(%d,%d,%d) k %d v %d\n", blockIdx.x, blockIdx.y, blockIdx.z, nk, nv);
-          __trap();
-        }
+      int g0 = 0, i = 0;
+      for (int u = u_first; u < u_end; u += u_step, ++i) {
+        const Unit w = unit_at(u);
+        const int n = w.ke - w.kb;
+        bool q_done = false;
+        int nk = 0, nv = 0;
+        uint32_t spins = 0;
+        while (!q_done || nk < n || nv < n) {
+          bool progress = false;
+          if (!q_done && (i == 0 || mbar_test(q_empty, (i - 1) & 1))) {
+            arm(q_full, Cfg::Q_TILE);
+#pragma unroll
+            for (int hh = 0; hh < HD / 64; ++hh)
+              load2(sQ + hh * Cfg::Q_HALF, &tmQ, q_full, w.h * HD + hh * 64, w.b * p.Nq + w.q_tile * TQ);
+            q_done = true;
+            progress = true;
+          }
+          const int gk = g0 + nk, gv = g0 + nv;
+          if (nk < n && mbar_test(&s_full[gk & 1], ((gk >> 1) & 1) ^ 1)) {
+            uint8_t* dst = sK + (gk & 1) * Cfg::K_TILE;
+            arm(&k_full[gk & 1], Cfg::K_TILE);
+#pragma unroll
+            for (int hh = 0; hh < HD / 64; ++hh)
+              load2(dst + hh * Cfg::K_HALF, &tmK, &k_full[gk & 1], w.h * HD + hh * 64,
+                    w.b * p.Nk + (w.kb + nk) * TK + static_cast<int>(rank) * Cfg::KROWS);
+            ++nk;
+            progress = true;
+          }
+          if (nv < n && mbar_test(&v_empty[gv & 1], ((gv >> 1) & 1) ^ 1)) {
+            arm(&v_full[gv & 1], Cfg::V_TILE);
+            if (PAIR)
+              tma_load_3d_2sm(sV + (gv & 1) * Cfg::V_TILE, &tmV, &v_full[gv & 1], (w.kb + nv) * TK,
+                              w.h * HD + static_cast<int>(rank) * Cfg::VROWS, w.b);
+            else
+              tma_load_3d(sV + (gv & 1) * Cfg::V_TILE, &tmV, &v_full[gv & 1], (w.kb + nv) * TK, w.h * HD, w.b);
+            ++nv;
+            progress = true;
+          }
+          if (progress) {
+            spins = 0;
+          } else if (__nanosleep(128), ++spins > (1u << 23)) {
+            printf("ltxcuda: attention producer stuck block(%d,%d,%d) unit %d k %d v %d\n", blockIdx.x, blockIdx.y, blockIdx.z, u, nk, nv);
+            __trap();
+          }
+        }
+        g0 += n;
       }
     }
   } else if (warp == 1) {
@@ -169,9 +216,9 @@
       for (int kk = 0; kk < TK / 16; ++kk)
 #pragma unroll
         for (int st = 0; st < 2; ++st) vd[st][kk] = umma_desc_sw128(smem_u32(sV + st * Cfg::V_TILE) + kk * 32);
-      auto issue_S = [&](int j, auto st_tag) {
+      auto issue_S = [&](int g, auto st_tag) {
         constexpr int st = decltype(st_tag)::value;
-        mbar_wait(&k_full[st], (j >> 1) & 1);
+        mbar_wait(&k_full[st], (g >> 1) & 1);
         tc_fence_after();
 #pragma unroll
         for (int kk = 0; kk < HD / 16; ++kk) {
@@ -180,30 +227,40 @@
         }
         commit(&s_full[st]);
       };
-      auto issue_PV = [&](int j, auto st_tag) {
+      auto issue_PV = [&](int g, bool first, auto st_tag) {
         constexpr int st = decltype(st_tag)::value;
-        mbar_wait(&v_full[st], (j >> 1) & 1);
-        mbar_wait(&p_full[st], (j >> 1) & 1);
+        mbar_wait(&v_full[st], (g >> 1) & 1);
+        mbar_wait(&p_full[st], (g >> 1) & 1);
         tc_fence_after();
 #pragma unroll
         for (int kk = 0; kk < TK / 16; ++kk) {
-          if (PAIR) umma_bf16_ts_2cta(tmem_base + 2 * TK, tmem_base + st * TK + kk * 8, vd[st][kk], idesc_o, (j | kk) != 0);
-          else umma_bf16_ts(tmem_base + 2 * TK, tmem_base + st * TK + kk * 8, vd[st][kk], idesc_o, (j | kk) != 0);
+          if (PAIR) umma_bf16_ts_2cta(tmem_base + 2 * TK, tmem_base + st * TK + kk * 8, vd[st][kk], idesc_o, (!first || kk != 0) ? 1u : 0u);
+          else umma_bf16_ts(tmem_base + 2 * TK, tmem_base + st * TK + kk * 8, vd[st][kk], idesc_o, (!first || kk != 0) ? 1u : 0u);
         }
         commit(&v_empty[st]);
       };
-      using S0 = std::integral_constant<int, 0>;
-      using S1 = std::integral_constant<int, 1>;
-      mbar_wait(q_full, 0);
-      issue_S(0, S0{});
-      if (n_kv > 1) issue_S(1, S1{});
-      for (int j = 0; j < n_kv; j += 2) {
-        issue_PV(j, S0{});
-        if (j + 2 < n_kv) issue_S(j + 2, S0{});
-        if (j + 1 < n_kv) {
-          issue_PV(j + 1, S1{});
-          if (j + 3 < n_kv) issue_S(j + 3, S1{});
-        }
+      auto run_unit = [&](int g0, int n, auto sa_tag) {
+        using SA = std::integral_constant<int, decltype(sa_tag)::value>;
+        using SB = std::integral_constant<int, decltype(sa_tag)::value ^ 1>;
+        issue_S(g0, SA{});
+        if (n > 1) issue_S(g0 + 1, SB{});
+        for (int j = 0; j < n; j += 2) {
+          issue_PV(g0 + j, j == 0, SA{});
+          if (j + 2 < n) issue_S(g0 + j + 2, SA{});
+          if (j + 1 < n) {
+            issue_PV(g0 + j + 1, false, SB{});
+            if (j + 3 < n) issue_S(g0 + j + 3, SB{});
+          }
+        }
+      };
+      int g0 = 0, i = 0;
+      for (int u = u_first; u < u_end; u += u_step, ++i) {
+        const Unit w = unit_at(u);
+        const int n = w.ke - w.kb;
+        mbar_wait(q_full, i & 1);
+        if (g0 & 1) run_unit(g0, n, std::integral_constant<int, 1>{});
+        else run_unit(g0, n, std::integral_constant<int, 0>{});
+        g0 += n;
       }
     }
   } else {
@@ -212,138 +269,229 @@
     const uint32_t lane_addr = static_cast<uint32_t>(q * 32) << 16;
     const uint32_t o_addr = tmem_base + lane_addr + 2 * TK;
     const float LOG2E = 1.4426950408889634f;
-    float m_ref = -1.0e30f, l_run = 0.f;
-    auto step = [&](int j, auto masked_tag) {
-      constexpr bool MASKED = decltype(masked_tag)::value;
-      const int st = j & 1;
-      const int kv0 = j * TK;
-      const int valid = min(TK, p.Nk - kv0);
-      const uint32_t s_addr = tmem_base + lane_addr + st * TK;
-      mbar_wait(&s_full[st], (j >> 1) & 1);
+    int g0 = 0;
+    for (int u = u_first; u < u_end; u += u_step) {
+      const Unit w = unit_at(u);
+      const int n = w.ke - w.kb;
+      float m_ref = -1.0e30f, l_run = 0.f;
+      auto step = [&](int j, auto masked_tag) {
+        constexpr bool MASKED = decltype(masked_tag)::value;
+        const int g = g0 + j;
+        const int st = g & 1;
+        const int kv0 = (w.kb + j) * TK;
+        const int valid = min(TK, p.Nk - kv0);
+        const uint32_t s_addr = tmem_base + lane_addr + st * TK;
+        mbar_wait(&s_full[st], (g >> 1) & 1);
+        tc_fence_after();
+        uint32_t sr[2][32];
+        tmem_ld32(s_addr, sr[0]);
+        tmem_ld32(s_addr + 32, sr[1]);
+        tmem_ld_wait();
+        float s[TK];
+#pragma unroll
+        for (int c = 0; c < 2; ++c)
+#pragma unroll
+          for (int i = 0; i < 32; ++i) s[c * 32 + i] = __uint_as_float(sr[c][i]);
+        if (MASKED && p.key_bias != nullptr) {
+          const float inv_scale = LOG2E / p.scale_log2;
+          const float* kb = p.key_bias + static_cast<int64_t>(w.b) * p.Nk + kv0;
+          if (valid == TK && (reinterpret_cast<uintptr_t>(kb) & 15) == 0) {
+#pragma unroll
+            for (int i = 0; i < TK; i += 4) {
+              const float4 bv = __ldg(reinterpret_cast<const float4*>(kb + i));
+              s[i] = fmaf(bv.x, inv_scale, s[i]);
+              s[i + 1] = fmaf(bv.y, inv_scale, s[i + 1]);
+              s[i + 2] = fmaf(bv.z, inv_scale, s[i + 2]);
+              s[i + 3] = fmaf(bv.w, inv_scale, s[i + 3]);
+            }
+          } else {
+#pragma unroll
+            for (int i = 0; i < TK; ++i)
+              if (i < valid) s[i] = fmaf(__ldg(kb + i), inv_scale, s[i]);
+          }
+        }
+        if (MASKED && valid < TK) {
+#pragma unroll
+          for (int i = 0; i < TK; ++i)
+            if (i >= valid) s[i] = -INFINITY;
+        }
+        float mx8[8];
+#pragma unroll
+        for (int i = 0; i < 8; ++i) mx8[i] = s[i];
+#pragma unroll
+        for (int i = 8; i < TK; ++i) mx8[i & 7] = fmaxf(mx8[i & 7], s[i]);
+        const float mx = fmaxf(fmaxf(fmaxf(mx8[0], mx8[1]), fmaxf(mx8[2], mx8[3])), fmaxf(fmaxf(mx8[4], mx8[5]), fmaxf(mx8[6], mx8[7])));
+        const float m_new = fmaxf(m_ref, mx);
+        const bool need = (m_new - m_ref) * p.scale_log2 > RESCALE_THRESHOLD;
+        if (__any_sync(0xffffffffu, need)) {
+          const float alpha = need ? ex2_approx((m_ref - m_new) * p.scale_log2) : 1.0f;
+          if (j > 0) {
+            mbar_wait(&v_empty[(g - 1) & 1], ((g - 1) >> 1) & 1);
+            tc_fence_after();
+            uint32_t r[32];
+#pragma unroll 1
+            for (int c = 0; c < HD / 32; ++c) {
+              tmem_ld32(o_addr + c * 32, r);
+              tmem_ld_wait();
+#pragma unroll
+              for (int i = 0; i < 32; ++i) r[i] = __float_as_uint(__uint_as_float(r[i]) * alpha);
+              tmem_st32(o_addr + c * 32, r);
+            }
+          }
+          l_run *= alpha;
+          if (need) m_ref = m_new;
+        }
+        const float neg = -m_ref * p.scale_log2;
+        float rs0 = 0.f, rs1 = 0.f;
+        uint32_t pk[32];
+#pragma unroll
+        for (int t = 0; t < 32; ++t) {
+          const float p0 = ex2_approx(fmaf(s[2 * t], p.scale_log2, neg));
+          const float p1 = ex2_approx(fmaf(s[2 * t + 1], p.scale_log2, neg));
+          rs0 += p0;
+          rs1 += p1;
+          pk[t] = pack_bf16(p0, p1);
+        }
+        tmem_st32(s_addr, pk);
+        l_run += rs0 + rs1;
+        tmem_st_wait();
+        tc_fence_before();
+        __syncwarp();
+        if (lane == 0) {
+          if (PAIR) mbar_arrive_remote(&p_full[st], 0);
+          else mbar_arrive(&p_full[st]);
+        }
+      };
+      {
+        const bool ragged = (p.Nk % TK) != 0 && w.ke == n_kv;
+        if (p.key_bias != nullptr) {
+          for (int j = 0; j < n; ++j) step(j, std::true_type{});
+        } else {
+          const int n_full = ragged ? n - 1 : n;
+          for (int j = 0; j < n_full; ++j) step(j, std::false_type{});
+          if (ragged) step(n - 1, std::true_type{});
+        }
+      }
+      const int g_last = g0 + n - 1;
+      g0 += n;
+      if (!PAIR && p.splits > 1) {
+        __syncwarp();
+        if (lane == 0) mbar_arrive(q_empty);
+      }
+      mbar_wait(&v_empty[g_last & 1], (g_last >> 1) & 1);
       tc_fence_after();
-      uint32_t sr[2][32];
-      tmem_ld32(s_addr, sr[0]);
-      tmem_ld32(s_addr + 32, sr[1]);
-      tmem_ld_wait();
-      float s[TK];
-#pragma unroll
-      for (int c = 0; c < 2; ++c)
-#pragma unroll
-        for (int i = 0; i < 32; ++i) s[c * 32 + i] = __uint_as_float(sr[c][i]);
-      if (MASKED && p.key_bias != nullptr) {
-        const float inv_scale = LOG2E / p.scale_log2;
-        const float* kb = p.key_bias + static_cast<int64_t>(b) * p.Nk + kv0;
-        if (valid == TK && (reinterpret_cast<uintptr_t>(kb) & 15) == 0) {
-#pragma unroll
-          for (int i = 0; i < TK; i += 4) {
-            const float4 bv = __ldg(reinterpret_cast<const float4*>(kb + i));
-            s[i] = fmaf(bv.x, inv_scale, s[i]);
-            s[i + 1] = fmaf(bv.y, inv_scale, s[i + 1]);
-            s[i + 2] = fmaf(bv.z, inv_scale, s[i + 2]);
-            s[i + 3] = fmaf(bv.w, inv_scale, s[i + 3]);
-          }
-        } else {
-#pragma unroll
-          for (int i = 0; i < TK; ++i)
-            if (i < valid) s[i] = fmaf(__ldg(kb + i), inv_scale, s[i]);
-        }
-      }
-      if (MASKED && valid < TK) {
-#pragma unroll
-        for (int i = 0; i < TK; ++i)
-          if (i >= valid) s[i] = -INFINITY;
-      }
-      float mx8[8];
-#pragma unroll
-      for (int i = 0; i < 8; ++i) mx8[i] = s[i];
-#pragma unroll
-      for (int i = 8; i < TK; ++i) mx8[i & 7] = fmaxf(mx8[i & 7], s[i]);
-      const float mx = fmaxf(fmaxf(fmaxf(mx8[0], mx8[1]), fmaxf(mx8[2], mx8[3])), fmaxf(fmaxf(mx8[4], mx8[5]), fmaxf(mx8[6], mx8[7])));
-      const float m_new = fmaxf(m_ref, mx);
-      const bool need = (m_new - m_ref) * p.scale_log2 > RESCALE_THRESHOLD;
-      if (__any_sync(0xffffffffu, need)) {
-        const float alpha = need ? ex2_approx((m_ref - m_new) * p.scale_log2) : 1.0f;
-        if (j > 0) {
-          mbar_wait(&v_empty[(j - 1) & 1], ((j - 1) >> 1) & 1);
-          tc_fence_after();
+      auto out_row = [&](int rr) -> bf16* {
+        const int qi = w.q_tile * TQ + rr;
+        if (qi >= p.Nq) return nullptr;
+        if (p.o_rows_per_block > 0)
+          return reinterpret_cast<bf16*>(p.o_blocks.p[qi / p.o_rows_per_block]) + static_cast<int64_t>(qi % p.o_rows_per_block) * p.ldo + w.h * HD;
+        return p.O + (static_cast<int64_t>(w.b) * p.Nq + qi) * p.ldo + w.h * HD;
+      };
+      if (PAIR || p.splits == 1) {
+        const float inv = 1.0f / l_run;
+        constexpr int ROW_BYTES = HD * 2, CPR = HD / 8;
+        uint8_t* otile = sQ;
+#pragma unroll 1
+        for (int c = 0; c < HD / 32; ++c) {
           uint32_t r[32];
+          tmem_ld32(o_addr + c * 32, r);
+          tmem_ld_wait();
+#pragma unroll
+          for (int i = 0; i < 32; i += 8) {
+            uint4 pkv = make_uint4(pack_bf16(__uint_as_float(r[i]) * inv, __uint_as_float(r[i + 1]) * inv),
+                                   pack_bf16(__uint_as_float(r[i + 2]) * inv, __uint_as_float(r[i + 3]) * inv),
+                                   pack_bf16(__uint_as_float(r[i + 4]) * inv, __uint_as_float(r[i + 5]) * inv),
+                                   pack_bf16(__uint_as_float(r[i + 6]) * inv, __uint_as_float(r[i + 7]) * inv));
+            const int chunk = c * 4 + (i >> 3);
+            *reinterpret_cast<uint4*>(otile + r_in * ROW_BYTES + ((chunk ^ (r_in & 7)) << 4)) = pkv;
+          }
+        }
+        __syncwarp();
+        constexpr int RPI = 32 / CPR;
+        const int sub = lane / CPR, ch = lane % CPR;
+#pragma unroll 4
+        for (int i = 0; i < 32 / RPI; ++i) {
+          const int rr = q * 32 + RPI * i + sub;
+          bf16* orow = out_row(rr);
+          if (orow == nullptr) continue;
+          *reinterpret_cast<uint4*>(orow + ch * 8) = *reinterpret_cast<const uint4*>(otile + rr * ROW_BYTES + ((ch ^ (rr & 7)) << 4));
+        }
+        if (!PAIR) {
+          fence_proxy_async_smem();
+          __syncwarp();
+          if (lane == 0) mbar_arrive(q_empty);
+        }
+      } else {
+        const int tile_id = (w.b * p.H + w.h) * p.tiles + w.q_tile;
+        float* part0 = p.partials + static_cast<size_t>(tile_id) * p.splits * part_floats<HD>();
+        float* part = part0 + static_cast<size_t>(w.seg) * part_floats<HD>();
+#pragma unroll 1
+        for (int c = 0; c < HD / 32; ++c) {
+          uint32_t r[32];
+          tmem_ld32(o_addr + c * 32, r);
+          tmem_ld_wait();
+#pragma unroll
+          for (int i = 0; i < 8; ++i)
+            __stcg(reinterpret_cast<float4*>(part) + (c * 8 + i) * TQ + r_in,
+                   make_float4(__uint_as_float(r[4 * i]), __uint_as_float(r[4 * i + 1]), __uint_as_float(r[4 * i + 2]),
+                               __uint_as_float(r[4 * i + 3])));
+        }
+        __stcg(part + HD * TQ + r_in, m_ref);
+        __stcg(part + HD * TQ + TQ + r_in, l_run);
+        __threadfence();
+        asm volatile("bar.sync 1, 128;" ::: "memory");
+        if (threadIdx.x == 64) *ticket = atomicAdd(p.tickets + tile_id, 1u);
+        asm volatile("bar.sync 1, 128;" ::: "memory");
+        if (*ticket == static_cast<uint32_t>(p.splits - 1)) {
+          __threadfence();
+          float mk[MAX_SPLITS], wk[MAX_SPLITS];
+          float m_max = -INFINITY;
+#pragma unroll
+          for (int k = 0; k < MAX_SPLITS; ++k)
+            if (k < p.splits) {
+              mk[k] = __ldcg(part0 + k * part_floats<HD>() + HD * TQ + r_in);
+              m_max = fmaxf(m_max, mk[k]);
+            }
+          float l_sum = 0.f;
+#pragma unroll
+          for (int k = 0; k < MAX_SPLITS; ++k)
+            if (k < p.splits) {
+              wk[k] = ex2_approx((mk[k] - m_max) * p.scale_log2);
+              l_sum = fmaf(wk[k], __ldcg(part0 + k * part_floats<HD>() + HD * TQ + TQ + r_in), l_sum);
+            }
+          const float inv = 1.0f / l_sum;
+          bf16* orow = out_row(r_in);
 #pragma unroll 1
           for (int c = 0; c < HD / 32; ++c) {
-            tmem_ld32(o_addr + c * 32, r);
-            tmem_ld_wait();
-#pragma unroll
-            for (int i = 0; i < 32; ++i) r[i] = __float_as_uint(__uint_as_float(r[i]) * alpha);
-            tmem_st32(o_addr + c * 32, r);
-          }
-        }
-        l_run *= alpha;
-        if (need) m_ref = m_new;
+            float4 acc[8];
+#pragma unroll
+            for (int i = 0; i < 8; ++i) acc[i] = make_float4(0.f, 0.f, 0.f, 0.f);
+#pragma unroll
+            for (int k = 0; k < MAX_SPLITS; ++k)
+              if (k < p.splits) {
+                const float4* src = reinterpret_cast<const float4*>(part0 + k * part_floats<HD>()) + c * 8 * TQ + r_in;
+                float4 t[8];
+#pragma unroll
+                for (int i = 0; i < 8; ++i) t[i] = __ldcg(src + i * TQ);
+#pragma unroll
+                for (int i = 0; i < 8; ++i) {
+                  acc[i].x = fmaf(wk[k], t[i].x, acc[i].x);
+                  acc[i].y = fmaf(wk[k], t[i].y, acc[i].y);
+                  acc[i].z = fmaf(wk[k], t[i].z, acc[i].z);
+                  acc[i].w = fmaf(wk[k], t[i].w, acc[i].w);
+                }
+              }
+            if (orow != nullptr) {
+#pragma unroll
+              for (int i = 0; i < 8; i += 2)
+                *reinterpret_cast<uint4*>(orow + c * 32 + i * 4) =
+                    make_uint4(pack_bf16(acc[i].x * inv, acc[i].y * inv), pack_bf16(acc[i].z * inv, acc[i].w * inv),
+                               pack_bf16(acc[i + 1].x * inv, acc[i + 1].y * inv), pack_bf16(acc[i + 1].z * inv, acc[i + 1].w * inv));
+            }
+          }
+          if (threadIdx.x == 64) p.tickets[tile_id] = 0;
+        }
       }
-      const float neg = -m_ref * p.scale_log2;
-      float rs0 = 0.f, rs1 = 0.f;
-      uint32_t pk[32];
-#pragma unroll
-      for (int t = 0; t < 32; ++t) {
-        const float p0 = ex2_approx(fmaf(s[2 * t], p.scale_log2, neg));
-        const float p1 = ex2_approx(fmaf(s[2 * t + 1], p.scale_log2, neg));
-        rs0 += p0;
-        rs1 += p1;
-        pk[t] = pack_bf16(p0, p1);
-      }
-      tmem_st32(s_addr, pk);
-      l_run += rs0 + rs1;
-      tmem_st_wait();
-      tc_fence_before();
-      __syncwarp();
-      if (lane == 0) {
-        if (PAIR) mbar_arrive_remote(&p_full[st], 0);
-        else mbar_arrive(&p_full[st]);
-      }
-    };
-    {
-      const bool ragged = (p.Nk % TK) != 0;
-      if (p.key_bias != nullptr) {
-        for (int j = 0; j < n_kv; ++j) step(j, std::true_type{});
-      } else {
-        const int n_full = ragged ? n_kv - 1 : n_kv;
-        for (int j = 0; j < n_full; ++j) step(j, std::false_type{});
-        if (ragged) step(n_kv - 1, std::true_type{});
-      }
-    }
-    mbar_wait(&v_empty[(n_kv - 1) & 1], ((n_kv - 1) >> 1) & 1);
-    tc_fence_after();
-    const float inv = 1.0f / l_run;
-    constexpr int ROW_BYTES = HD * 2, CPR = HD / 8;
-    uint8_t* otile = sQ;
-#pragma unroll 1
-    for (int c = 0; c < HD / 32; ++c) {
-      uint32_t r[32];
-      tmem_ld32(o_addr + c * 32, r);
-      tmem_ld_wait();
-#pragma unroll
-      for (int i = 0; i < 32; i += 8) {
-        uint4 pkv = make_uint4(pack_bf16(__uint_as_float(r[i]) * inv, __uint_as_float(r[i + 1]) * inv),
-                               pack_bf16(__uint_as_float(r[i + 2]) * inv, __uint_as_float(r[i + 3]) * inv),
-                               pack_bf16(__uint_as_float(r[i + 4]) * inv, __uint_as_float(r[i + 5]) * inv),
-                               pack_bf16(__uint_as_float(r[i + 6]) * inv, __uint_as_float(r[i + 7]) * inv));
-        const int chunk = c * 4 + (i >> 3);
-        *reinterpret_cast<uint4*>(otile + r_in * ROW_BYTES + ((chunk ^ (r_in & 7)) << 4)) = pkv;
-      }
-    }
-    __syncwarp();
-    constexpr int RPI = 32 / CPR;
-    const int sub = lane / CPR, ch = lane % CPR;
-#pragma unroll 4
-    for (int i = 0; i < 32 / RPI; ++i) {
-      const int rr = q * 32 + RPI * i + sub;
-      const int qi = q_tile * TQ + rr;
-      if (qi >= p.Nq) continue;
-      const uint4 v = *reinterpret_cast<const uint4*>(otile + rr * ROW_BYTES + ((ch ^ (rr & 7)) << 4));
-      bf16* orow = p.O + (static_cast<int64_t>(b) * p.Nq + qi) * p.ldo + h * HD;
-      if (p.o_rows_per_block > 0)
-        orow = reinterpret_cast<bf16*>(p.o_blocks.p[qi / p.o_rows_per_block]) +
-               static_cast<int64_t>(qi % p.o_rows_per_block) * p.ldo + h * HD;
-      *reinterpret_cast<uint4*>(orow + ch * 8) = v;
     }
   }
   tc_fence_before();
@@ -358,7 +506,7 @@
 }
 
 template <int HD, bool PAIR>
-void attention_launch(const bf16* Q, int64_t ldq, const bf16* K, int64_t ldk, const bf16* Vt, int64_t ldvb, const AttnParams& p,
+void attention_launch(const bf16* Q, int64_t ldq, const bf16* K, int64_t ldk, const bf16* Vt, int64_t ldvb, AttnParams p,
                       int D, cudaStream_t stream) {
   using Cfg = AttCfg<HD, PAIR>;
   auto kern = attention_fwd_tcgen05<HD, PAIR>;
@@ -366,9 +514,15 @@
   CUtensorMap tmQ = make_tmap_2d(Q, static_cast<uint64_t>(p.B) * p.Nq, D, ldq, 128);
   CUtensorMap tmK = make_tmap_2d(K, static_cast<uint64_t>(p.B) * p.Nk, D, ldk, Cfg::KROWS);
   CUtensorMap tmV = make_tmap_3d(Vt, p.Nk, D, p.B, static_cast<uint64_t>(p.B) * ldvb, ldvb, TK, Cfg::VROWS);
-  int tiles = (p.Nq + TQ - 1) / TQ;
-  if (PAIR) tiles = (tiles + 1) & ~1;
-  dim3 grid(tiles, p.H, p.B);
+  dim3 grid;
+  if (PAIR) {
+    p.splits = 1;
+    p.units = 1;
+    grid = dim3((p.tiles + 1) & ~1, p.H, p.B);
+  } else {
+    p.units = p.B * p.H * p.tiles * p.splits;
+    grid = dim3(std::min(p.units, 2 * device_sm_count()));
+  }
   cudaLaunchConfig_t cfg = {};
   cfg.gridDim = grid;
   cfg.blockDim = dim3(ATT_THREADS);
@@ -391,11 +545,34 @@
   LTX_CUDA(cudaLaunchKernelEx(&cfg, kern, tmQ, tmK, tmV, p));
 }
 
+bool use_pair(int Nq) {
+  const char* pair_str = getenv("LTX_ATT_PAIR");
+  const int pair_env = pair_str ? atoi(pair_str) : -1;
+  return pair_env < 0 ? Nq >= 3072 : (pair_env != 0 && Nq > TQ);
+}
+
+int attention_splits(int Nk) {
+  const int n_kv = (Nk + TK - 1) / TK;
+  const char* s_env = getenv("LTX_ATT_SPLIT");
+  if (s_env) return std::max(1, std::min(std::min(atoi(s_env), MAX_SPLITS), n_kv));
+  return std::max(1, std::min((n_kv + 4) / 8, MAX_SPLITS));
+}
+
+}
+
+AttnWsSize attention_workspace_size(int B, int H, int Nq, int Nk, int head_dim) {
+  AttnWsSize s;
+  const int splits = use_pair(Nq) ? 1 : attention_splits(Nk);
+  if (splits == 1) return s;
+  const size_t tiles = static_cast<size_t>(B) * H * ((Nq + TQ - 1) / TQ);
+  s.ticket_bytes = tiles * sizeof(unsigned int);
+  s.partial_bytes = tiles * splits * (head_dim == 128 ? part_floats<128>() : part_floats<64>()) * sizeof(float);
+  return s;
 }
 
 void launch_attention(const bf16* Q, int64_t ldq, const bf16* K, int64_t ldk, const bf16* Vt, int64_t ldvb,
                       const float* key_bias, bf16* O, int64_t ldo, int B, int H, int Nq, int Nk, int D, float scale,
-                      cudaStream_t stream, const PeerTable* o_blocks, int rows_per_block) {
+                      const AttnWs& ws, cudaStream_t stream, const PeerTable* o_blocks, int rows_per_block) {
   LTX_CHECK(D == H * 128 || D == H * 64, 2, "attention: head_dim must be 128 or 64");
   LTX_CHECK(Nq > 0 && Nk > 0 && B > 0, 2, "attention: empty problem");
   LTX_CHECK(ldvb % 8 == 0 && ldvb >= Nk, 2, "attention: V^T per-batch pitch must be a multiple of 8 and >= Nk");
@@ -412,9 +589,14 @@
     p.o_rows_per_block = rows_per_block;
     p.o_blocks = *o_blocks;
   }
-  const char* pair_str = getenv("LTX_ATT_PAIR");
-  const int pair_env = pair_str ? atoi(pair_str) : -1;
-  const bool pair = pair_env < 0 ? Nq >= 3072 : (pair_env != 0 && Nq > TQ);
+  const bool pair = use_pair(Nq);
+  p.tiles = (Nq + TQ - 1) / TQ;
+  p.splits = pair ? 1 : attention_splits(Nk);
+  p.units = 0;
+  p.tickets = ws.tickets;
+  p.partials = ws.partials;
+  LTX_CHECK(p.splits == 1 || (ws.tickets != nullptr && ws.partials != nullptr), 2,
+            "attention: a split launch needs the context's workspace (attention_workspace_size)");
   if (D == H * 128) {
     if (pair) attention_launch<128, true>(Q, ldq, K, ldk, Vt, ldvb, p, D, stream);
     else attention_launch<128, false>(Q, ldq, K, ldk, Vt, ldvb, p, D, stream);
diff --git a/ltx-video-swift-mlx_b200/csrc/ctx.h b/ltx-video-swift-mlx_b200/csrc/ctx.h
--- a/ltx-video-swift-mlx_b200/csrc/ctx.h
+++ b/ltx-video-swift-mlx_b200/csrc/ctx.h
@@ -210,6 +210,7 @@
   int quant_materialise = 0;
   ltx::DevBuf q_panel;
   ltx::DevBuf gemm_ws;
+  ltx::DevBuf attn_tickets, attn_part;
   std::vector<void*> owned;
   bool dit_ready = false;
   std::vector<ltx::BlockWeights> blocks;
@@ -258,6 +259,7 @@
 
 namespace ltx {
 void gemm_attach_workspace(ltx_ctx* c, GemmEpi& e);
+AttnWs attention_workspace(ltx_ctx* c, int B, int H, int Nq, int Nk, int head_dim);
 struct ProfScope {
   ltx_ctx* c;
   ProfRec r;
diff --git a/ltx-video-swift-mlx_b200/csrc/dit.cu b/ltx-video-swift-mlx_b200/csrc/dit.cu
--- a/ltx-video-swift-mlx_b200/csrc/dit.cu
+++ b/ltx-video-swift-mlx_b200/csrc/dit.cu
@@ -44,7 +44,8 @@
                const PeerTable* o_blocks = nullptr, int rows_per_block = 0) {
   ProfScope ps(c, PROF_ATTN, 4.0 * B * H * static_cast<double>(Nq) * Nk * 128.0,
                2.0 * B * (2.0 * Nq + 2.0 * Nk) * D);
-  launch_attention(Q, ldq, K, ldk, Vt, ldvb, bias, O, ldo, B, H, Nq, Nk, D, scale, c->stream, o_blocks, rows_per_block);
+  launch_attention(Q, ldq, K, ldk, Vt, ldvb, bias, O, ldo, B, H, Nq, Nk, D, scale, attention_workspace(c, B, H, Nq, Nk, D / H),
+                   c->stream, o_blocks, rows_per_block);
 }
 void norm_mod(ltx_ctx* c, const float* x, bf16* out, int M, int D, const float* ts, const float* tsc, const float* as,
               const float* asc, int64_t ada_ld, int rows_per_mod, float eps, int ln) {
@@ -218,6 +219,19 @@
   e.ws_counter_count = kCounters;
   e.ws = reinterpret_cast<float*>(c->gemm_ws.as<uint8_t>() + kCounters * 4);
   e.ws_bytes = kPartials;
+}
+
+AttnWs attention_workspace(ltx_ctx* c, int B, int H, int Nq, int Nk, int head_dim) {
+  const AttnWsSize need = attention_workspace_size(B, H, Nq, Nk, head_dim);
+  if (need.ticket_bytes > c->attn_tickets.bytes) {
+    c->attn_tickets.reserve(need.ticket_bytes);
+    LTX_CUDA(cudaMemsetAsync(c->attn_tickets.ptr, 0, c->attn_tickets.bytes, c->stream));
+  }
+  c->attn_part.reserve(need.partial_bytes);
+  AttnWs ws;
+  ws.tickets = c->attn_tickets.as<unsigned int>();
+  ws.partials = c->attn_part.as<float>();
+  return ws;
 }
 
 void dit_clear_caches(ltx_ctx* c) {
diff --git a/ltx-video-swift-mlx_b200/csrc/dit_av.cu b/ltx-video-swift-mlx_b200/csrc/dit_av.cu
--- a/ltx-video-swift-mlx_b200/csrc/dit_av.cu
+++ b/ltx-video-swift-mlx_b200/csrc/dit_av.cu
@@ -250,7 +250,8 @@
                int hd, int B, int Nq, int Nk) {
   const int D = H * hd;
   ProfScope ps(c, PROF_ATTN, 4.0 * B * H * static_cast<double>(Nq) * Nk * hd, 2.0 * B * (2.0 * Nq + 2.0 * Nk) * D);
-  launch_attention(Q, D, K, ldk, Vt, ldv, bias, O, D, B, H, Nq, Nk, D, 1.0f / sqrtf(static_cast<float>(hd)), c->stream);
+  launch_attention(Q, D, K, ldk, Vt, ldv, bias, O, D, B, H, Nq, Nk, D, 1.0f / sqrtf(static_cast<float>(hd)),
+                   attention_workspace(c, B, H, Nq, Nk, hd), c->stream);
 }
 void normw(ltx_ctx* c, const float* x, bf16* out, int M, int D, const float* w, const float* sc_t, const float* sc_a,
            const float* sh_t, const float* sh_a, float eps, int64_t a_ld = 0, int a_rpr = 1) {
@@ -582,7 +583,8 @@
     }
     {
       ProfScope ps(c, PROF_ATTN, 4.0 * B * Hv * static_cast<double>(N) * N * hdv, 2.0 * 4.0 * R * D);
-      launch_attention(qk, 2 * D, qk + D, 2 * D, vt, ldv, nullptr, att, D, B, Hv, N, N, D, 1.0f / sqrtf(static_cast<float>(hdv)), st);
+      launch_attention(qk, 2 * D, qk + D, 2 * D, vt, ldv, nullptr, att, D, B, Hv, N, N, D, 1.0f / sqrtf(static_cast<float>(hdv)),
+                       attention_workspace(c, B, Hv, N, N, hdv), st);
     }
     linear_resid(c, att, R, D, bv.a1.wo, bv.a1.bo, D, x, vada + 2 * D, bv.sst + 2 * D, vada_ld, v_rpr, B);
     normw(c, ax, ah, Ra, Da, ba.anorm1, ba.asst + Da, aada + Da, ba.asst, aada, eps, aada_ld, Ta);
diff --git a/ltx-video-swift-mlx_b200/csrc/ltx_internal.h b/ltx-video-swift-mlx_b200/csrc/ltx_internal.h
--- a/ltx-video-swift-mlx_b200/csrc/ltx_internal.h
+++ b/ltx-video-swift-mlx_b200/csrc/ltx_internal.h
@@ -132,9 +132,17 @@
 CUtensorMap make_tmap_u8(const void* base, uint64_t rows, uint64_t row_bytes, uint32_t box_rows, uint32_t box_bytes);
 void launch_transpose_bf16(const bf16* in, int64_t ld_in, int R, int C, bf16* out, int64_t ld_out, cudaStream_t s);
 
+struct AttnWs {
+  unsigned int* tickets = nullptr;
+  float* partials = nullptr;
+};
+struct AttnWsSize {
+  size_t ticket_bytes = 0, partial_bytes = 0;
+};
+AttnWsSize attention_workspace_size(int B, int H, int Nq, int Nk, int head_dim);
 void launch_attention(const bf16* Q, int64_t ldq, const bf16* K, int64_t ldk, const bf16* Vt, int64_t ldvb,
                       const float* key_bias, bf16* O, int64_t ldo, int B, int H, int Nq, int Nk, int D, float scale,
-                      cudaStream_t stream, const PeerTable* o_blocks = nullptr, int rows_per_block = 0);
+                      const AttnWs& ws, cudaStream_t stream, const PeerTable* o_blocks = nullptr, int rows_per_block = 0);
 
 void launch_rmsnorm_mod(const float* x, bf16* out, int M, int D, const float* tbl_shift, const float* tbl_scale,
                         const float* ada_shift, const float* ada_scale, int64_t ada_ld, int rows_per_mod, float eps,
```

Measured after the change: 23.99 (median of 6 runs). 0.935x the previous value.
